# JCZ404/Semi-DETR

Hardware: AMD Instinct MI355X
Metric: images/sec/node DINO-R50 SSOD step (hot path: MSDA fwd/bwd + Hungarian + EMA/pseudo-label) (higher is better)
Workload: dtype f32

## Files before the change

include/semidetr_hip.h:

```cpp
#ifndef SEMIDETR_HIP_H
#define SEMIDETR_HIP_H

#include <stddef.h>
#include <stdint.h>

#ifdef __cplusplus
extern "C" {
#endif

#define SEMIDETR_OK 0
#define SEMIDETR_E_BADARG (-1)
#define SEMIDETR_E_TOOLARGE (-2)
#define SEMIDETR_E_NODEVICE (-3)

#define SEMIDETR_ABI_VERSION 7

int semidetr_abi_version(void);
const char *semidetr_last_error(void);

#define SEMIDETR_MSDA_QUERIES_ARE_PIXELS 1
#define SEMIDETR_MSDA_POLICY_SLOT(s) (((s) & 0xff) << 8)
#define SEMIDETR_MSDA_FIXED_FORWARD 2
#define SEMIDETR_MSDA_GATHER_WINDOW (1 << 16)
#define SEMIDETR_MSDA_GATHER_PATCH (1 << 17)
int semidetr_msda_forward_f32(void *stream, const float *value, const int64_t *spatial_shapes,
                              const int64_t *level_start, const float *sampling_loc,
                              const float *attn_weight, int batch, int spatial_size, int num_heads,
                              int channels, int num_levels, int num_query, int num_point, int flags, float *out);
int semidetr_msda_forward_f64(void *stream, const double *value, const int64_t *spatial_shapes,
                              const int64_t *level_start, const double *sampling_loc,
                              const double *attn_weight, int batch, int spatial_size, int num_heads,
                              int channels, int num_levels, int num_query, int num_point, double *out);
int semidetr_msda_backward_f32(void *stream, const float *grad_out, const float *value,
                               const int64_t *spatial_shapes, const int64_t *level_start,
                               const float *sampling_loc, const float *attn_weight, int batch,
                               int spatial_size, int num_heads, int channels, int num_levels,
                               int num_query, int num_point, int flags, float *grad_value,
                               float *grad_sampling_loc, float *grad_attn_weight);
int semidetr_msda_backward_f64(void *stream, const double *grad_out, const double *value,
                               const int64_t *spatial_shapes, const int64_t *level_start,
                               const double *sampling_loc, const double *attn_weight, int batch,
                               int spatial_size, int num_heads, int channels, int num_levels,
                               int num_query, int num_point, double *grad_value,
                               double *grad_sampling_loc, double *grad_attn_weight);

int semidetr_msda_fused_forward_f32(void *stream, const float *value, const int64_t *spatial_shapes,
                                    const int64_t *level_start, const float *reference_points, int ref_dim,
                                    const float *sampling_offsets, const float *attn_logits,
                                    const unsigned char *padding_mask, const int *mask_extents, int batch,
                                    int spatial_size, int num_heads, int channels, int num_levels,
                                    int num_query, int num_point, int flags, float *out);
int semidetr_msda_fused_backward_f32(void *stream, const float *grad_out, const float *value,
                                     const int64_t *spatial_shapes, const int64_t *level_start,
                                     const float *reference_points, int ref_dim,
                                     const float *sampling_offsets, const float *attn_logits,
                                     const unsigned char *padding_mask, const int *mask_extents, int batch,
                                     int spatial_size, int num_heads, int channels, int num_levels,
                                     int num_query, int num_point, int flags, float *grad_value,
                                     float *grad_sampling_offsets, float *grad_attn_logits);
int semidetr_msda_forward_f32_v2(void *stream, const float *value, const int64_t *spatial_shapes,
                                 const int64_t *level_start, const float *sampling_loc,
                                 const float *attn_weight, int batch, int spatial_size, int num_heads,
                                 int channels, int num_levels, int num_query, int num_point, int flags, float *out,
                                 const int64_t *host_spatial_shapes);
int semidetr_msda_backward_f32_v2(void *stream, const float *grad_out, const float *value,
                                  const int64_t *spatial_shapes, const int64_t *level_start,
                                  const float *sampling_loc, const float *attn_weight, int batch,
                                  int spatial_size, int num_heads, int channels, int num_levels,
                                  int num_query, int num_point, int flags, float *grad_value,
                                  float *grad_sampling_loc, float *grad_attn_weight, const int64_t *host_spatial_shapes);
int semidetr_msda_fused_forward_f32_v2(void *stream, const float *value, const int64_t *spatial_shapes,
                                       const int64_t *level_start, const float *reference_points, int ref_dim,
                                       const float *sampling_offsets, const float *attn_logits,
                                       const unsigned char *padding_mask, const int *mask_extents, int batch,
                                       int spatial_size, int num_heads, int channels, int num_levels,
                                       int num_query, int num_point, int flags, float *out,
                                       const int64_t *host_spatial_shapes);
int semidetr_msda_fused_backward_f32_v2(void *stream, const float *grad_out, const float *value,
                                        const int64_t *spatial_shapes, const int64_t *level_start,
                                        const float *reference_points, int ref_dim,
                                        const float *sampling_offsets, const float *attn_logits,
                                        const unsigned char *padding_mask, const int *mask_extents, int batch,
                                        int spatial_size, int num_heads, int channels, int num_levels,
                                        int num_query, int num_point, int flags, float *grad_value,
                                        float *grad_sampling_offsets, float *grad_attn_logits,
                                        const int64_t *host_spatial_shapes);
int semidetr_msda_mask_extents(void *stream, const unsigned char *padding_mask, const int64_t *spatial_shapes,
                               const int64_t *level_start, int batch, int spatial_size, int num_levels, int *extents);

int semidetr_msda_set_forward_policy(int policy);
int semidetr_msda_forward_policy_state(int *policy, int *mode, float *far_fraction, unsigned *updates);
int semidetr_msda_forward_policy_state_slot(int slot, int *policy, int *mode, float *far_fraction, unsigned *updates);
int semidetr_msda_gather_choice(int slot);

#define SEMIDETR_MSDA_GRID_FORWARD 0
#define SEMIDETR_MSDA_GRID_GATHER 1
#define SEMIDETR_MSDA_GRID_SCATTER 2
int semidetr_msda_set_region_grid(int kernel, int nry, int nrx);
int semidetr_msda_region_grid_query(int kernel, const int64_t *host_spatial_shapes, int num_levels, int batch, int num_heads,
                                    int num_cus, int *grid6);

const char *semidetr_msda_last_kernels(void);

#define SEMIDETR_H16_FP16 0
#define SEMIDETR_H16_BF16 1
int semidetr_msda_forward_h16(void *stream, int dtype, const void *value, const int64_t *spatial_shapes,
                              const int64_t *level_start, const float *sampling_loc, const float *attn_weight,
                              int batch, int spatial_size, int num_heads, int channels, int num_levels, int num_query,
                              int num_point, void *out);
size_t semidetr_msda_backward_h16_workspace_bytes(int batch, int spatial_size, int num_heads, int channels);
int semidetr_msda_backward_h16(void *stream, int dtype, const void *grad_out, const void *value,
                               const int64_t *spatial_shapes, const int64_t *level_start, const float *sampling_loc,
                               const float *attn_weight, int batch, int spatial_size, int num_heads, int channels,
                               int num_levels, int num_query, int num_point, void *workspace, void *grad_value,
                               float *grad_sampling_loc, float *grad_attn_weight);
int semidetr_msda_fused_forward_h16(void *stream, int dtype, const void *value, const int64_t *spatial_shapes,
                                    const int64_t *level_start, const float *reference_points, int ref_dim,
                                    const void *sampling_offsets, const void *attn_logits, int prologue_type,
                                    const unsigned char *padding_mask, int batch, int spatial_size, int num_heads,
                                    int channels, int num_levels, int num_query, int num_point, void *out);
int semidetr_msda_fused_backward_h16(void *stream, int dtype, const void *grad_out, const void *value,
                                     const int64_t *spatial_shapes, const int64_t *level_start,
                                     const float *reference_points, int ref_dim, const void *sampling_offsets,
                                     const void *attn_logits, int prologue_type, const unsigned char *padding_mask,
                                     int batch, int spatial_size, int num_heads, int channels, int num_levels,
                                     int num_query, int num_point, void *workspace, void *grad_value,
                                     void *grad_sampling_offsets, void *grad_attn_logits);
const char *semidetr_msda_h16_last_kernels(void);

typedef struct semidetr_cost_params {
    float cls_weight;
    float alpha;
    float gamma;
    float eps;
    float reg_weight;
    int   reg_xywh;
    float iou_weight;
    int   iou_giou;
    int   pred_xyxy;
} semidetr_cost_params;

int semidetr_match_cost_f32(void *stream, const float *bbox_pred, const float *cls_pred,
                            const float *gt_bboxes, const int64_t *gt_labels,
                            const int32_t *gt_offsets, const float *img_wh, int num_problems,
                            int num_query, int num_classes, int total_gt,
                            const semidetr_cost_params *params , float *cost);

int64_t semidetr_lsap_workspace_bytes(int num_problems, int num_query, int max_gt);
int semidetr_lsap_solve(void *stream, const float *cost, const int32_t *gt_offsets,
                        const int64_t *gt_labels, int num_problems, int num_query, int total_gt,
                        int max_gt, int64_t *match_row, int64_t *match_col,
                        int64_t *assigned_gt_inds, int64_t *assigned_labels, int32_t *status,
                        void *workspace);

int semidetr_build_targets(void *stream, const int64_t *assigned_gt_inds, const float *gt_bboxes,
                           const int64_t *gt_labels, const int32_t *gt_offsets, const float *img_wh,
                           int num_problems, int num_query, int64_t num_classes, int64_t *labels,
                           float *label_weights, float *bbox_targets, float *bbox_weights, int32_t *num_pos);

#define SEMIDETR_EMA_CHUNK 8192
int semidetr_ema_multi_f32(void *stream, float *const *teacher_ptrs, const float *const *student_ptrs,
                           const int64_t *numels, const int32_t *block_starts, int num_tensors,
                           int total_blocks, double momentum);
int semidetr_ema_flat_f32(void *stream, float *teacher, const float *student, int64_t numel,
                          double momentum);

int semidetr_pseudo_label_filter_f32(void *stream, const float *proposals, const int64_t *labels,
                                     const int32_t *prop_offsets, const int32_t *prop_counts,
                                     int num_images, float *out_boxes,
                                     int64_t *out_labels, float *out_scores, int32_t *out_keep_idx,
                                     int32_t *out_count, float *out_thr);

size_t semidetr_nms_workspace_bytes(int batch, int num_query, int num_classes);
int semidetr_pseudo_nms_f32(void *stream, const float *cls_logits, const float *bbox_pred, const float *img_hw,
                            int batch, int num_query, int num_classes, float score_thr, float iou_thr,
                            int max_per_img, void *workspace, size_t workspace_bytes, float *out_dets,
                            int64_t *out_labels, int32_t *out_count);

int semidetr_transform_bboxes_f32(void *stream, const float *boxes, int box_stride, const int32_t *box_offsets,
                                  const int32_t *box_counts, int num_images, int max_boxes_per_image,
                                  const float *matrices, const float *out_hw, float *out_boxes);

int semidetr_o2m_assign_f32(void *stream, const float *bbox_pred, const float *cls_prob, const float *gt_bboxes,
                            const int64_t *gt_labels, const int32_t *gt_offsets, const float *img_wh,
                            int num_problems, int num_query, int num_classes, int total_gt,
                            int max_gt_per_problem, int candidate_topk, int dynamic_k, float alpha, float beta,
                            int64_t *gt_inds, int64_t *labels, float *max_overlaps, float *assign_metrics,
                            int64_t *labels_full, float *bbox_targets, float *norm_metrics);

size_t semidetr_tal_loss_workspace_bytes(void);
int semidetr_tal_loss_f32(void *stream, const float *logits, const int64_t *labels, const float *metrics,
                          int64_t num_rows, int num_classes, float gamma, int input_is_prob, void *workspace,
                          float *loss_sum, float *grad_logits);

#define SEMIDETR_GMM_COVARIANCE_DIAG 1
int semidetr_gmm_match_costs_f32(void *stream, const float *cost, const int32_t *gt_offsets, const int32_t *pair_offsets,
                                 const int64_t *rows, const int64_t *cols, int num_images, int num_query, int num_pairs,
                                 int capacity, float *out_seg, int32_t *out_count);
int semidetr_gmm_fit_f64(void *stream, const float *values, int64_t value_stride, const int32_t *counts,
                         int64_t count_stride, int num_segments, int capacity, int covariance_type, double reg_covar,
                         double tol, int max_iter, float *out_thr, int32_t *out_labels, double *out_scores,
                         int32_t *out_info);
int semidetr_gmm_double_filter_f32(void *stream, const float *seg_costs, const int32_t *pair_offsets, const int64_t *cols,
                                   const float *thr, const float *gt_bboxes, const int64_t *gt_labels,
                                   const float *gt_scores, const float *det_bboxes, const int64_t *det_labels,
                                   const float *det_scores, const int32_t *gt_offsets, int num_images, int max_gt,
                                   float base_thr, int slot, float *out_base_boxes, int64_t *out_base_labels,
                                   float *out_base_scores, float *out_gmm_boxes, int64_t *out_gmm_labels,
                                   float *out_gmm_scores, float *out_det_boxes, int64_t *out_det_labels,
                                   float *out_det_scores, int32_t *out_counts);

#define SEMIDETR_SET_LOSS_MATCHED 0
#define SEMIDETR_SET_LOSS_DN 1
#define SEMIDETR_SET_LOSS_WARMUP 2
#define SEMIDETR_SET_LOSS_MAX_SEGMENTS 3
#define SEMIDETR_SET_LOSS_MAX_LAYERS 64
#define SEMIDETR_SET_LOSS_NUM_STATS 10
#define SEMIDETR_SET_LOSS_NUM_TERMS 5
typedef struct semidetr_set_loss_segment {
    int kind, num_layers, num_images, num_query, num_classes;
    const float *logits;
    int64_t logit_stride[3];
    const float *boxes;
    int64_t box_stride[3];
    const int64_t *labels;
    const float *label_weights, *bbox_targets, *bbox_weights, *metrics;
    const int32_t *gt_offsets;
    const float *gt_boxes;
    const int64_t *gt_labels;
    int single_pad, dn_groups;
    const float *img_wh;
    float alpha, gamma, cls_weight, l1_weight, iou_weight, iou_eps, bg_cls_weight;
    int sync_cls;
    float *grad_logits, *grad_boxes;
} semidetr_set_loss_segment;
int64_t semidetr_set_loss_workspace_bytes(const semidetr_set_loss_segment *segs, int num_segments);
int semidetr_set_loss_forward_f32(void *stream, const semidetr_set_loss_segment *segs, int num_segments, void *workspace,
                                  int64_t workspace_bytes, double *stats, float *norms, float *losses, float *scales);
int semidetr_set_loss_finalize_f32(void *stream, const semidetr_set_loss_segment *segs, int num_segments,
                                   const double *stats, const float *norms_local, const float *norms_reduced,
                                   float *losses, float *scales);
int semidetr_set_loss_backward_f32(void *stream, const semidetr_set_loss_segment *segs, int num_segments,
                                   const float *scales, const float *grad_out);

#define SEMIDETR_DN_MAX_IMAGES 64
#define SEMIDETR_DN_NOISE_COLS 10
typedef struct semidetr_dn_layout {
    int num_images, single_pad, groups;
    int32_t offsets[SEMIDETR_DN_MAX_IMAGES + 1];
} semidetr_dn_layout;
typedef struct semidetr_dn_build {
    semidetr_dn_layout dn, cons;
    int32_t src_counts[SEMIDETR_DN_MAX_IMAGES];
    const int64_t *labels[SEMIDETR_DN_MAX_IMAGES];
    const float *boxes[SEMIDETR_DN_MAX_IMAGES];
    int box_stride, num_known;
    const float *label_weight;
    int num_embeddings, hidden_dim, num_classes, num_queries;
    const float *noise, *image_noise;
    float label_noise_threshold, box_noise_scale;
    float *query_label, *query_bbox;
    int64_t *known_bid, *map_known_indice, *noised_labels, *pad_mask;
    const float *cons_rows;
    float *cons_label;
    unsigned char *attn_mask;
} semidetr_dn_build;
typedef struct semidetr_dn_consistency {
    semidetr_dn_layout cons;
    int32_t src_counts[SEMIDETR_DN_MAX_IMAGES];
    const float *pseudo_boxes[SEMIDETR_DN_MAX_IMAGES];
    const float *det_boxes[SEMIDETR_DN_MAX_IMAGES];
    int pseudo_stride, det_stride, num_known;
    float tgt_wh[SEMIDETR_DN_MAX_IMAGES][2], src_wh[SEMIDETR_DN_MAX_IMAGES][2];
    float *query_bbox, *known_bid;
    int64_t *map_known_indice;
    float *loss_weights, *rois;
    float loss_weight;
} semidetr_dn_consistency;
int semidetr_dn_build_f32(void *stream, const semidetr_dn_build *params );
int semidetr_dn_consistency_f32(void *stream, const semidetr_dn_consistency *params );
int semidetr_dn_label_backward_f32(void *stream, const float *grad_query_label, const int64_t *known_bid,
                                   const int64_t *map_known_indice, const int64_t *noised_labels, int num_known,
                                   int num_images, int pad_size, int hidden_dim, int num_embeddings, float *grad_weight);
int semidetr_dn_gather_rows_f32(void *stream, const semidetr_dn_layout *layout , const float *grad_label,
                                int hidden_dim, float *grad_rows);

#define SEMIDETR_QSEL_MAX_LEVELS 8
#define SEMIDETR_QSEL_MAX_K 4096
int semidetr_qsel_proposals_f32(void *stream, const float *memory, const unsigned char *padding_mask,
                                const int64_t *spatial_shapes_host, const int64_t *spatial_shapes_dev, int num_levels, int N,
                                int S, int D, float *output_memory, float *output_proposals, unsigned char *valid);
int semidetr_qsel_proposals_backward_f32(void *stream, const float *grad_output_memory, const unsigned char *valid, int N, int S,
                                         int D, float *grad_memory);
size_t semidetr_qsel_topk_workspace_bytes(int N, int S);
int semidetr_qsel_topk_f32(void *stream, const float *logits, int N, int S, int C, int k, void *workspace,
                           size_t workspace_bytes, int64_t *indices, int32_t *inverse);
int semidetr_qsel_gather_f32(void *stream, const int64_t *indices, const float *coord, const float *proposals,
                             const float *memory, int N, int S, int k, int D, float *refpoint, float *init_box, float *tgt,
                             float *ref_enc);
int semidetr_qsel_gather_backward_f32(void *stream, const int32_t *inverse, const float *grad_refpoint, const float *grad_tgt,
                                      const float *grad_ref_enc, const float *ref_enc, int N, int S, int k, int D,
                                      float *grad_coord, float *grad_memory);

#define SEMIDETR_DET_MAX_K 2048
size_t semidetr_det_workspace_bytes(int batch, int num_query, int num_classes, int k);
int semidetr_det_decode_f32(void *stream, const float *cls_logits, const float *bbox_pred, const float *img_hw,
                            const float *scale_factor , int batch, int num_query,
                            int num_classes, int k, void *workspace, size_t workspace_bytes, float *out_dets ,
                            int64_t *out_labels , float *out_dets_by_class ,
                            int32_t *out_class_offsets );

#define SEMIDETR_CONSIS_MAX_LAYERS 16
typedef struct semidetr_consis_layer {
    const float *v1, *v2;
    int64_t v1_stride[2], v2_stride[2];
    float *grad_v1;
} semidetr_consis_layer;
typedef struct semidetr_consis_loss {
    int num_layers, batch, num_query, dim, pad_size, num_known;
    int bid_is_int64;
    float scale, eps;
    const void *known_bid;
    const int64_t *map_known_indice;
    const float *loss_weights;
    semidetr_consis_layer layer[SEMIDETR_CONSIS_MAX_LAYERS];
} semidetr_consis_loss;
size_t semidetr_consis_loss_workspace_bytes(int num_layers, int num_known, int batch, int pad_size);
int semidetr_consis_loss_forward_f32(void *stream, const semidetr_consis_loss *params , void *workspace,
                                     size_t workspace_bytes, float *losses);
int semidetr_consis_loss_backward_f32(void *stream, const semidetr_consis_loss *params , const void *workspace,
                                      size_t workspace_bytes, const float *grad_losses);

typedef struct semidetr_self_attn {
    int batch, heads, head_dim, len_q, len_k;
    float scale;
    const float *q, *k, *v;
    int64_t q_stride[2], k_stride[2], v_stride[2];
    const uint8_t *mask;
    float *out, *lse;
    const float *grad_out;
    float *grad_q, *grad_k, *grad_v;
    int64_t gq_stride[2], gk_stride[2], gv_stride[2];
} semidetr_self_attn;
size_t semidetr_self_attn_workspace_bytes(int batch, int heads, int len_q, int len_k);
int semidetr_self_attn_forward_f32(void *stream, const semidetr_self_attn *params , void *workspace,
                                   size_t workspace_bytes);
int semidetr_self_attn_backward_f32(void *stream, const semidetr_self_attn *params , void *workspace,
                                    size_t workspace_bytes);

typedef struct semidetr_self_attn_h16 {
    int batch, heads, head_dim, len_q, len_k;
    float scale;
    int type;
    const void *q, *k, *v;
    int64_t q_stride[2], k_stride[2], v_stride[2];
    const uint8_t *mask;
    void *out;
    float *lse;
    const void *grad_out;
    void *grad_q, *grad_k, *grad_v;
    int64_t gq_stride[2], gk_stride[2], gv_stride[2];
} semidetr_self_attn_h16;
int semidetr_self_attn_forward_h16(void *stream, const semidetr_self_attn_h16 *params , void *workspace,
                                   size_t workspace_bytes);
int semidetr_self_attn_backward_h16(void *stream, const semidetr_self_attn_h16 *params , void *workspace,
                                    size_t workspace_bytes);

typedef struct semidetr_add_norm {
    int rows0, rows1, dim;
    float eps;
    const float *x, *residual, *pos;
    const float *gy, *gq;
    int64_t x_stride[2], residual_stride[2], pos_stride[2], gy_stride[2], gq_stride[2];
    const float *weight, *bias;
    float *y, *q;
    float *mean, *rstd;
    float *grad_x, *grad_weight, *grad_bias;
} semidetr_add_norm;
size_t semidetr_add_norm_workspace_bytes(int64_t rows);
int semidetr_add_norm_forward_f32(void *stream, const semidetr_add_norm *params , void *workspace,
                                  size_t workspace_bytes);
int semidetr_add_norm_backward_f32(void *stream, const semidetr_add_norm *params , void *workspace,
                                   size_t workspace_bytes);

#define SEMIDETR_ROW_F32 0
#define SEMIDETR_ROW_FP16 1
#define SEMIDETR_ROW_BF16 2
typedef struct semidetr_add_norm_mixed {
    int rows0, rows1, dim;
    float eps;
    const void *x, *residual, *pos;
    const void *gy, *gq;
    int64_t x_stride[2], residual_stride[2], pos_stride[2], gy_stride[2], gq_stride[2];
    const float *weight, *bias;
    void *y, *q;
    float *mean, *rstd;
    void *grad_x, *grad_residual, *grad_pos;
    float *grad_weight, *grad_bias;
    int x_type, residual_type, pos_type, gy_type, gq_type;
    int y_type, q_type, grad_x_type, grad_residual_type, grad_pos_type;
} semidetr_add_norm_mixed;
int semidetr_add_norm_forward_mixed(void *stream, const semidetr_add_norm_mixed *params , void *workspace,
                                    size_t workspace_bytes);
int semidetr_add_norm_backward_mixed(void *stream, const semidetr_add_norm_mixed *params , void *workspace,
                                     size_t workspace_bytes);

#define SEMIDETR_GN_MAX_LEVELS 8
typedef struct semidetr_gn_tokens {
    int batch, levels, channels, groups;
    float eps;
    int64_t hw[SEMIDETR_GN_MAX_LEVELS], start[SEMIDETR_GN_MAX_LEVELS];
    int64_t tokens_per_image;
    const void *x[SEMIDETR_GN_MAX_LEVELS];
    int64_t x_batch_stride[SEMIDETR_GN_MAX_LEVELS];
    const float *weight[SEMIDETR_GN_MAX_LEVELS], *bias[SEMIDETR_GN_MAX_LEVELS];
    void *grad_x[SEMIDETR_GN_MAX_LEVELS];
    float *grad_weight[SEMIDETR_GN_MAX_LEVELS], *grad_bias[SEMIDETR_GN_MAX_LEVELS];
    void *tokens, *q;
    const void *pos, *gy, *gq;
    int64_t pos_stride[2], gy_stride[2], gq_stride[2];
    float *mean, *rstd;
    int x_type, out_type, pos_type;
} semidetr_gn_tokens;
size_t semidetr_gn_tokens_workspace_bytes(const semidetr_gn_tokens *params , int for_backward);
int semidetr_gn_tokens_forward(void *stream, const semidetr_gn_tokens *params , void *workspace,
                               size_t workspace_bytes);
int semidetr_gn_tokens_backward(void *stream, const semidetr_gn_tokens *params , void *workspace,
                                size_t workspace_bytes);

#define SEMIDETR_REF_MAX_SEGMENTS 8
#define SEMIDETR_REF_MAX_LEVELS 8
#define SEMIDETR_REF_NONE 0
#define SEMIDETR_REF_SIGMOID 1
#define SEMIDETR_REF_REFINE 2
typedef struct semidetr_ref_segment {
    int rows0, rows1;
    const void *delta, *ref;
    int64_t delta_stride[2], ref_stride[2];
    void *new_ref;
    int64_t new_ref_stride[2];
    const void *g_new;
    int64_t g_new_stride[2];
    void *g_delta, *g_ref;
} semidetr_ref_segment;
typedef struct semidetr_ref_points {
    int width, mode, num_segments, levels;
    float eps;
    int delta_type, ref_type, out_type;
    const float *valid_ratios;
    const float *dim_t;
    float *ref_input;
    float *embed;
    const float *g_ref_input, *g_embed;
    semidetr_ref_segment segment[SEMIDETR_REF_MAX_SEGMENTS];
} semidetr_ref_points;
int semidetr_ref_points_forward(void *stream, const semidetr_ref_points *params );
int semidetr_ref_points_backward(void *stream, const semidetr_ref_points *params );

#ifdef __cplusplus
}
#endif
#endif
```

semi-detr_amd/_lib.py:

```python
import contextlib
import ctypes
import os

import torch

_HERE = os.path.dirname(os.path.abspath(__file__))
EXPERIMENTS = os.environ.get("SEMIDETR_EXPERIMENTS", "0") not in ("", "0")
LIB_PATH = os.path.join(_HERE, "csrc", "libsemidetr_hip_exp.so" if EXPERIMENTS else "libsemidetr_hip.so")

c_void_p, c_int, c_int64, c_double = ctypes.c_void_p, ctypes.c_int, ctypes.c_int64, ctypes.c_double
c_float, c_size_t, POINTER = ctypes.c_float, ctypes.c_size_t, ctypes.POINTER

CONSTANTS = {
    "SEMIDETR_ABI_VERSION": 7,
    "SEMIDETR_EMA_CHUNK": 8192,
    "SEMIDETR_GMM_COVARIANCE_DIAG": 1,
    "SEMIDETR_SET_LOSS_MATCHED": 0, "SEMIDETR_SET_LOSS_DN": 1, "SEMIDETR_SET_LOSS_WARMUP": 2,
    "SEMIDETR_SET_LOSS_MAX_LAYERS": 64, "SEMIDETR_SET_LOSS_NUM_STATS": 10, "SEMIDETR_SET_LOSS_NUM_TERMS": 5,
    "SEMIDETR_DN_MAX_IMAGES": 64, "SEMIDETR_DN_NOISE_COLS": 10,
    "SEMIDETR_QSEL_MAX_LEVELS": 8, "SEMIDETR_QSEL_MAX_K": 4096,
    "SEMIDETR_DET_MAX_K": 2048,
    "SEMIDETR_CONSIS_MAX_LAYERS": 16,
}
ROW_TYPES = {"SEMIDETR_ROW_F32": 0, "SEMIDETR_ROW_FP16": 1, "SEMIDETR_ROW_BF16": 2}
_DN_IMAGES, _CONSIS_LAYERS = CONSTANTS["SEMIDETR_DN_MAX_IMAGES"], CONSTANTS["SEMIDETR_CONSIS_MAX_LAYERS"]
_STRIDE2 = c_int64 * 2


def _f(ctype, names):
    return [(n, ctype) for n in names.split()]


class CostParams(ctypes.Structure):
    _fields_ = (_f(c_float, "cls_weight alpha gamma eps reg_weight") + _f(c_int, "reg_xywh") + _f(c_float, "iou_weight")
                + _f(c_int, "iou_giou pred_xyxy"))


class SetLossSegment(ctypes.Structure):
    _fields_ = (_f(c_int, "kind num_layers num_images num_query num_classes")
                + _f(c_void_p, "logits") + _f(c_int64 * 3, "logit_stride") + _f(c_void_p, "boxes") + _f(c_int64 * 3, "box_stride")
                + _f(c_void_p, "labels label_weights bbox_targets bbox_weights metrics gt_offsets gt_boxes gt_labels")
                + _f(c_int, "single_pad dn_groups") + _f(c_void_p, "img_wh")
                + _f(c_float, "alpha gamma cls_weight l1_weight iou_weight iou_eps bg_cls_weight") + _f(c_int, "sync_cls")
                + _f(c_void_p, "grad_logits grad_boxes"))


class DnLayout(ctypes.Structure):
    _fields_ = _f(c_int, "num_images single_pad groups") + _f(ctypes.c_int32 * (_DN_IMAGES + 1), "offsets")


class DnBuild(ctypes.Structure):
    _fields_ = (_f(DnLayout, "dn cons") + _f(ctypes.c_int32 * _DN_IMAGES, "src_counts") + _f(c_void_p * _DN_IMAGES, "labels boxes")
                + _f(c_int, "box_stride num_known") + _f(c_void_p, "label_weight")
                + _f(c_int, "num_embeddings hidden_dim num_classes num_queries") + _f(c_void_p, "noise image_noise")
                + _f(c_float, "label_noise_threshold box_noise_scale")
                + _f(c_void_p, "query_label query_bbox known_bid map_known_indice noised_labels pad_mask cons_rows cons_label "
                               "attn_mask"))


class DnConsistency(ctypes.Structure):
    _fields_ = (_f(DnLayout, "cons") + _f(ctypes.c_int32 * _DN_IMAGES, "src_counts")
                + _f(c_void_p * _DN_IMAGES, "pseudo_boxes det_boxes") + _f(c_int, "pseudo_stride det_stride num_known")
                + _f(c_float * 2 * _DN_IMAGES, "tgt_wh src_wh")
                + _f(c_void_p, "query_bbox known_bid map_known_indice loss_weights rois") + _f(c_float, "loss_weight"))


class ConsisLayer(ctypes.Structure):
    _fields_ = _f(c_void_p, "v1 v2") + _f(_STRIDE2, "v1_stride v2_stride") + _f(c_void_p, "grad_v1")


class ConsisLoss(ctypes.Structure):
    _fields_ = (_f(c_int, "num_layers batch num_query dim pad_size num_known bid_is_int64") + _f(c_float, "scale eps")
                + _f(c_void_p, "known_bid map_known_indice loss_weights") + _f(ConsisLayer * _CONSIS_LAYERS, "layer"))


class SelfAttn(ctypes.Structure):
    _fields_ = (_f(c_int, "batch heads head_dim len_q len_k") + _f(c_float, "scale") + _f(c_void_p, "q k v")
                + _f(_STRIDE2, "q_stride k_stride v_stride") + _f(c_void_p, "mask out lse grad_out grad_q grad_k grad_v")
                + _f(_STRIDE2, "gq_stride gk_stride gv_stride"))


class SelfAttnH16(ctypes.Structure):
    _fields_ = (_f(c_int, "batch heads head_dim len_q len_k") + _f(c_float, "scale") + _f(c_int, "type") + _f(c_void_p, "q k v")
                + _f(_STRIDE2, "q_stride k_stride v_stride") + _f(c_void_p, "mask out lse grad_out grad_q grad_k grad_v")
                + _f(_STRIDE2, "gq_stride gk_stride gv_stride"))


class AddNorm(ctypes.Structure):
    _fields_ = (_f(c_int, "rows0 rows1 dim") + _f(c_float, "eps") + _f(c_void_p, "x residual pos gy gq")
                + _f(_STRIDE2, "x_stride residual_stride pos_stride gy_stride gq_stride")
                + _f(c_void_p, "weight bias y q mean rstd grad_x grad_weight grad_bias"))


class AddNormMixed(ctypes.Structure):
    _fields_ = (_f(c_int, "rows0 rows1 dim") + _f(c_float, "eps") + _f(c_void_p, "x residual pos gy gq")
                + _f(_STRIDE2, "x_stride residual_stride pos_stride gy_stride gq_stride")
                + _f(c_void_p, "weight bias y q mean rstd grad_x grad_residual grad_pos grad_weight grad_bias")
                + _f(c_int, "x_type residual_type pos_type gy_type gq_type y_type q_type grad_x_type grad_residual_type "
                            "grad_pos_type"))


GN_MAX_LEVELS = 8
_GN_I64, _GN_PTR = c_int64 * GN_MAX_LEVELS, c_void_p * GN_MAX_LEVELS


class GnTokens(ctypes.Structure):
    _fields_ = (_f(c_int, "batch levels channels groups") + _f(c_float, "eps") + _f(_GN_I64, "hw start")
                + _f(c_int64, "tokens_per_image") + _f(_GN_PTR, "x") + _f(_GN_I64, "x_batch_stride")
                + _f(_GN_PTR, "weight bias grad_x grad_weight grad_bias") + _f(c_void_p, "tokens q pos gy gq")
                + _f(_STRIDE2, "pos_stride gy_stride gq_stride") + _f(c_void_p, "mean rstd") + _f(c_int, "x_type out_type pos_type"))


REF_MAX_SEGMENTS, REF_MAX_LEVELS = 8, 8
REF_MODES = {"SEMIDETR_REF_NONE": 0, "SEMIDETR_REF_SIGMOID": 1, "SEMIDETR_REF_REFINE": 2}


class RefSegment(ctypes.Structure):
    _fields_ = (_f(c_int, "rows0 rows1") + _f(c_void_p, "delta ref") + _f(_STRIDE2, "delta_stride ref_stride")
                + _f(c_void_p, "new_ref") + _f(_STRIDE2, "new_ref_stride") + _f(c_void_p, "g_new") + _f(_STRIDE2, "g_new_stride")
                + _f(c_void_p, "g_delta g_ref"))


class RefPoints(ctypes.Structure):
    _fields_ = (_f(c_int, "width mode num_segments levels") + _f(c_float, "eps") + _f(c_int, "delta_type ref_type out_type")
                + _f(c_void_p, "valid_ratios dim_t ref_input embed g_ref_input g_embed")
                + _f(RefSegment * REF_MAX_SEGMENTS, "segment"))


STRUCTS = {"semidetr_cost_params": CostParams, "semidetr_set_loss_segment": SetLossSegment, "semidetr_dn_layout": DnLayout,
           "semidetr_dn_build": DnBuild, "semidetr_dn_consistency": DnConsistency, "semidetr_consis_layer": ConsisLayer,
           "semidetr_consis_loss": ConsisLoss, "semidetr_self_attn": SelfAttn, "semidetr_self_attn_h16": SelfAttnH16,
           "semidetr_add_norm": AddNorm,
           "semidetr_add_norm_mixed": AddNormMixed, "semidetr_gn_tokens": GnTokens,
           "semidetr_ref_segment": RefSegment, "semidetr_ref_points": RefPoints}
_SEGS, _WORK = POINTER(SetLossSegment), [c_void_p, c_size_t]

_MSDA_FWD = [c_void_p] * 6 + [c_int] * 7 + [c_void_p]
_MSDA_BWD = [c_void_p] * 7 + [c_int] * 7 + [c_void_p] * 3
_MSDA_FWD_F32 = [c_void_p] * 6 + [c_int] * 8 + [c_void_p]
_MSDA_BWD_F32 = [c_void_p] * 7 + [c_int] * 8 + [c_void_p] * 3

SIGNATURES = {
    "semidetr_abi_version": (c_int, []),
    "semidetr_last_error": (ctypes.c_char_p, []),
    "semidetr_msda_forward_f32": (c_int, _MSDA_FWD_F32),
    "semidetr_msda_forward_f64": (c_int, _MSDA_FWD),
    "semidetr_msda_backward_f32": (c_int, _MSDA_BWD_F32),
    "semidetr_msda_backward_f64": (c_int, _MSDA_BWD),
    "semidetr_msda_fused_forward_f32": (c_int, [c_void_p] * 5 + [c_int] + [c_void_p] * 4 + [c_int] * 8 + [c_void_p]),
    "semidetr_msda_fused_backward_f32": (c_int, [c_void_p] * 6 + [c_int] + [c_void_p] * 4 + [c_int] * 8 + [c_void_p] * 3),
    "semidetr_msda_forward_f32_v2": (c_int, _MSDA_FWD_F32 + [c_void_p]),
    "semidetr_msda_backward_f32_v2": (c_int, _MSDA_BWD_F32 + [c_void_p]),
    "semidetr_msda_fused_forward_f32_v2": (c_int, [c_void_p] * 5 + [c_int] + [c_void_p] * 4 + [c_int] * 8 + [c_void_p] * 2),
    "semidetr_msda_fused_backward_f32_v2": (c_int, [c_void_p] * 6 + [c_int] + [c_void_p] * 4 + [c_int] * 8 + [c_void_p] * 4),
    "semidetr_msda_mask_extents": (c_int, [c_void_p] * 4 + [c_int] * 3 + [c_void_p]),
    "semidetr_msda_last_kernels": (ctypes.c_char_p, []),
    "semidetr_msda_forward_h16": (c_int, [c_void_p, c_int] + [c_void_p] * 5 + [c_int] * 7 + [c_void_p]),
    "semidetr_msda_backward_h16_workspace_bytes": (c_size_t, [c_int] * 4),
    "semidetr_msda_backward_h16": (c_int, [c_void_p, c_int] + [c_void_p] * 6 + [c_int] * 7 + [c_void_p] * 4),
    "semidetr_msda_fused_forward_h16": (c_int, [c_void_p, c_int] + [c_void_p] * 4 + [c_int] + [c_void_p] * 2 + [c_int, c_void_p] +
                                        [c_int] * 7 + [c_void_p]),
    "semidetr_msda_fused_backward_h16": (c_int, [c_void_p, c_int] + [c_void_p] * 5 + [c_int] + [c_void_p] * 2 + [c_int, c_void_p] +
                                         [c_int] * 7 + [c_void_p] * 4),
    "semidetr_msda_h16_last_kernels": (ctypes.c_char_p, []),
    "semidetr_msda_set_forward_policy": (c_int, [c_int]),
    "semidetr_msda_forward_policy_state": (c_int, [c_void_p] * 4),
    "semidetr_msda_forward_policy_state_slot": (c_int, [c_int] + [c_void_p] * 4),
    "semidetr_msda_gather_choice": (c_int, [c_int]),
    "semidetr_msda_set_region_grid": (c_int, [c_int] * 3),
    "semidetr_msda_region_grid_query": (c_int, [c_int, c_void_p] + [c_int] * 4 + [c_void_p]),
    "semidetr_match_cost_f32": (c_int, [c_void_p] * 7 + [c_int] * 4 + [POINTER(CostParams), c_void_p]),
    "semidetr_lsap_workspace_bytes": (c_int64, [c_int, c_int, c_int]),
    "semidetr_lsap_solve": (c_int, [c_void_p] * 4 + [c_int] * 4 + [c_void_p] * 6),
    "semidetr_build_targets": (c_int, [c_void_p] * 6 + [c_int, c_int, c_int64] + [c_void_p] * 5),
    "semidetr_ema_multi_f32": (c_int, [c_void_p] * 5 + [c_int, c_int, c_double]),
    "semidetr_ema_flat_f32": (c_int, [c_void_p, c_void_p, c_void_p, c_int64, c_double]),
    "semidetr_pseudo_label_filter_f32": (c_int, [c_void_p] * 5 + [c_int] + [c_void_p] * 6),
    "semidetr_nms_workspace_bytes": (c_size_t, [c_int, c_int, c_int]),
    "semidetr_pseudo_nms_f32": (c_int, [c_void_p] * 4 + [c_int] * 3 + [c_float, c_float, c_int, c_void_p,
                                                                       c_size_t] + [c_void_p] * 3),
    "semidetr_o2m_assign_f32": (c_int, [c_void_p] * 7 + [c_int] * 7 + [c_float, c_float] + [c_void_p] * 7),
    "semidetr_tal_loss_workspace_bytes": (c_size_t, []),
    "semidetr_tal_loss_f32": (c_int, [c_void_p] * 4 + [c_int64, c_int, c_float, c_int] + [c_void_p] * 3),
    "semidetr_transform_bboxes_f32": (c_int, [c_void_p, c_void_p, c_int, c_void_p, c_void_p, c_int, c_int] + [c_void_p] * 3),
    "semidetr_gmm_match_costs_f32": (c_int, [c_void_p] * 6 + [c_int] * 4 + [c_void_p] * 2),
    "semidetr_gmm_fit_f64": (c_int, [c_void_p, c_void_p, c_int64, c_void_p, c_int64] + [c_int] * 3 + [c_double, c_double, c_int]
                             + [c_void_p] * 4),
    "semidetr_gmm_double_filter_f32": (c_int, [c_void_p] * 12 + [c_int, c_int, c_float, c_int] + [c_void_p] * 10),
    "semidetr_set_loss_workspace_bytes": (c_int64, [_SEGS, c_int]),
    "semidetr_set_loss_forward_f32": (c_int, [c_void_p, _SEGS, c_int, c_void_p, c_int64] + [c_void_p] * 4),
    "semidetr_set_loss_finalize_f32": (c_int, [c_void_p, _SEGS, c_int] + [c_void_p] * 5),
    "semidetr_set_loss_backward_f32": (c_int, [c_void_p, _SEGS, c_int, c_void_p, c_void_p]),
    "semidetr_dn_build_f32": (c_int, [c_void_p, POINTER(DnBuild)]),
    "semidetr_dn_consistency_f32": (c_int, [c_void_p, POINTER(DnConsistency)]),
    "semidetr_dn_label_backward_f32": (c_int, [c_void_p] * 5 + [c_int] * 5 + [c_void_p]),
    "semidetr_dn_gather_rows_f32": (c_int, [c_void_p, POINTER(DnLayout), c_void_p, c_int, c_void_p]),
    "semidetr_qsel_proposals_f32": (c_int, [c_void_p] * 5 + [c_int] * 4 + [c_void_p] * 3),
    "semidetr_qsel_proposals_backward_f32": (c_int, [c_void_p] * 3 + [c_int] * 3 + [c_void_p]),
    "semidetr_qsel_topk_workspace_bytes": (c_size_t, [c_int, c_int]),
    "semidetr_qsel_topk_f32": (c_int, [c_void_p, c_void_p] + [c_int] * 4 + [c_void_p, c_size_t, c_void_p, c_void_p]),
    "semidetr_qsel_gather_f32": (c_int, [c_void_p] * 5 + [c_int] * 4 + [c_void_p] * 4),
    "semidetr_qsel_gather_backward_f32": (c_int, [c_void_p] * 6 + [c_int] * 4 + [c_void_p] * 2),
    "semidetr_det_workspace_bytes": (c_size_t, [c_int] * 4),
    "semidetr_det_decode_f32": (c_int, [c_void_p] * 5 + [c_int] * 4 + [c_void_p, c_size_t] + [c_void_p] * 4),
    "semidetr_consis_loss_workspace_bytes": (c_size_t, [c_int] * 4),
    "semidetr_consis_loss_forward_f32": (c_int, [c_void_p, POINTER(ConsisLoss)] + _WORK + [c_void_p]),
    "semidetr_consis_loss_backward_f32": (c_int, [c_void_p, POINTER(ConsisLoss)] + _WORK + [c_void_p]),
    "semidetr_self_attn_workspace_bytes": (c_size_t, [c_int] * 4),
    "semidetr_self_attn_forward_f32": (c_int, [c_void_p, POINTER(SelfAttn)] + _WORK),
    "semidetr_self_attn_backward_f32": (c_int, [c_void_p, POINTER(SelfAttn)] + _WORK),
    "semidetr_self_attn_forward_h16": (c_int, [c_void_p, POINTER(SelfAttnH16)] + _WORK),
    "semidetr_self_attn_backward_h16": (c_int, [c_void_p, POINTER(SelfAttnH16)] + _WORK),
    "semidetr_add_norm_workspace_bytes": (c_size_t, [c_int64]),
    "semidetr_add_norm_forward_f32": (c_int, [c_void_p, POINTER(AddNorm)] + _WORK),
    "semidetr_add_norm_backward_f32": (c_int, [c_void_p, POINTER(AddNorm)] + _WORK),
    "semidetr_add_norm_forward_mixed": (c_int, [c_void_p, POINTER(AddNormMixed)] + _WORK),
    "semidetr_add_norm_backward_mixed": (c_int, [c_void_p, POINTER(AddNormMixed)] + _WORK),
    "semidetr_gn_tokens_workspace_bytes": (c_size_t, [POINTER(GnTokens), c_int]),
    "semidetr_gn_tokens_forward": (c_int, [c_void_p, POINTER(GnTokens)] + _WORK),
    "semidetr_gn_tokens_backward": (c_int, [c_void_p, POINTER(GnTokens)] + _WORK),
    "semidetr_ref_points_forward": (c_int, [c_void_p, POINTER(RefPoints)]),
    "semidetr_ref_points_backward": (c_int, [c_void_p, POINTER(RefPoints)]),
}

EXPERIMENT_SIGNATURES = {
    "semidetr_msda_set_variant": (None, [c_int, c_int]),
    "semidetr_debug_counters": (c_int, [c_void_p, c_int]),
    "semidetr_stream_copy_f32": (c_int, [c_void_p, c_void_p, c_void_p, c_int64, c_int]),
}

_lib = None


class NativeLibraryError(RuntimeError):
    pass


def lib():
    global _lib
    if _lib is None:
        if not os.path.exists(LIB_PATH):
            raise NativeLibraryError(
                f"{LIB_PATH} not found: build it with `python -c 'import __graft_entry__ as g; g.build()'` "
                "or `make -C semi-detr_amd/csrc` (hipcc --offload-arch=gfx950). There is no CPU fallback.")
        handle = ctypes.CDLL(LIB_PATH)
        table = dict(SIGNATURES, **EXPERIMENT_SIGNATURES) if EXPERIMENTS else SIGNATURES
        for name, (res, args) in table.items():
            fn = getattr(handle, name)
            fn.restype, fn.argtypes = res, args
        _lib = handle
    return _lib


def check(rc, what):
    if rc != 0:
        msg = lib().semidetr_last_error().decode(errors="replace")
        raise RuntimeError(f"{what} failed (code {rc}): {msg}")


def current_stream_ptr():
    return c_void_p(torch.cuda.current_stream().cuda_stream)


_NO_GUARD = contextlib.nullcontext()
_Tensor = torch.Tensor
_functions = {}


def device_guard(dev):
    if dev.index is None or dev.index == torch.cuda.current_device():
        return _NO_GUARD
    return torch.cuda.device(dev)


def ptr_args(args):
    return [c_void_p(a.data_ptr()) if isinstance(a, _Tensor) else a for a in args]


def _function(name):
    hit = _functions.get(name)
    if hit is not None and hit[0] is _lib:
        return hit[1]
    if name not in SIGNATURES and not (EXPERIMENTS and name in EXPERIMENT_SIGNATURES):
        raise AttributeError(f"{name} is not a function of the C ABI (_lib.SIGNATURES)")
    fn = getattr(lib(), name)
    _functions[name] = (_lib, fn)
    return fn


def calls(dev, *launches):
    fns = [_function(launch[0]) for launch in launches]
    with device_guard(dev):
        stream = c_void_p(torch.cuda.current_stream(dev).cuda_stream)
        for fn, launch in zip(fns, launches):
            rc = fn(stream, *ptr_args(launch[1:]))
            if rc:
                check(rc, launch[0])


def call(name, dev, *args):
    calls(dev, (name,) + args)


def small_to_device(values, dtype, dev):
    host = torch.tensor(values, dtype=dtype)
    if dev.type == "cuda":
        return host.pin_memory().to(dev, non_blocking=True)
    return host.to(dev)


def offsets(counts, dev):
    offs = [0]
    for c in counts:
        offs.append(offs[-1] + int(c))
    return offs, small_to_device(offs, torch.int32, dev)


def rows_f32(t):
    t = t.detach()
    if t.dtype != torch.float32:
        t = t.float()
    if t.stride(2) != 1 or t.data_ptr() % 16 or t.stride(0) % 4 or t.stride(1) % 4:
        t = t.contiguous()
    return t


def row_type(dtype):
    code = _ROW_TYPE_OF.get(dtype)
    if code is None:
        raise TypeError(f"rows of {dtype} are not built (float32, float16, bfloat16)")
    return code


_ROW_TYPE_OF = {torch.float32: ROW_TYPES["SEMIDETR_ROW_F32"], torch.float16: ROW_TYPES["SEMIDETR_ROW_FP16"],
                torch.bfloat16: ROW_TYPES["SEMIDETR_ROW_BF16"]}


def rows_native(t):
    t = t.detach()
    row_type(t.dtype)
    if t.stride(2) != 1 or t.data_ptr() % (16 if t.dtype == torch.float32 else 8) or t.stride(0) % 4 or t.stride(1) % 4:
        t = t.contiguous()
    return t


def set_rows(block, name, t, stride=None):
    if t is None:
        return
    setattr(block, name, t.data_ptr())
    st, strides = getattr(block, stride or name + "_stride"), t.stride()
    st[0], st[1] = strides[0], strides[1]


def cast(t, dtype):
    return t if t is None or t.dtype == dtype else t.to(dtype)


FORWARD_POLICIES = {"adaptive": 0, "patch": 1, "window": 2}


def set_forward_policy(policy):
    check(lib().semidetr_msda_set_forward_policy(FORWARD_POLICIES.get(policy, policy)), "semidetr_msda_set_forward_policy")


def forward_policy_state(slot=0):
    pol, mode, upd, frac = c_int(), c_int(), ctypes.c_uint(), c_float()
    check(lib().semidetr_msda_forward_policy_state_slot(int(slot), ctypes.byref(pol), ctypes.byref(mode), ctypes.byref(frac),
                                                        ctypes.byref(upd)), "semidetr_msda_forward_policy_state_slot")
    return {"policy": pol.value, "mode": mode.value, "far_fraction": frac.value, "updates": upd.value}


REGION_GRID_KERNELS = {"forward": 0, "gather": 1, "scatter": 2}


def set_region_grid(kernel, nry=0, nrx=0):
    check(lib().semidetr_msda_set_region_grid(REGION_GRID_KERNELS.get(kernel, kernel), int(nry), int(nrx)),
          "semidetr_msda_set_region_grid")


def region_grid(kernel, spatial_shapes, batch, num_heads, num_cus):
    flat = None if spatial_shapes is None else [int(v) for hw in spatial_shapes for v in hw]
    table = None if flat is None else (c_int64 * len(flat))(*flat)
    levels = 1 if flat is None else len(flat) // 2
    out = (c_int * 6)()
    check(lib().semidetr_msda_region_grid_query(REGION_GRID_KERNELS.get(kernel, kernel), table, levels, int(batch), int(num_heads),
                                                int(num_cus), out), "semidetr_msda_region_grid_query")
    return dict(zip(("nry", "nrx", "regions", "workgroups", "tail_split", "max_queries"), out))


def set_variant(fwd, bwd):
    if EXPERIMENTS:
        lib().semidetr_msda_set_variant(int(fwd), int(bwd))
    elif (fwd, bwd) != (0, 0):
        raise NativeLibraryError("kernel variants exist only in the experiments build: set SEMIDETR_EXPERIMENTS=1 "
                                 "(libsemidetr_hip_exp.so) before importing semi_detr_amd")
```

semi-detr_amd/csrc/lsap.hip:

```cpp
#include <hip/hip_runtime.h>

#include "common.h"

#pragma clang fp contract(off)

namespace {

constexpr double kInf = __builtin_huge_val();

struct Best {
    double low;
    int first;
    int last_un;
};

__device__ __forceinline__ Best combine(const Best &a, const Best &b)
{
    if (b.low < a.low) return b;
    if (a.low < b.low) return a;
    Best r = a;
    r.first = min(a.first, b.first);
    r.last_un = max(a.last_un, b.last_un);
    return r;
}

template <int CTRL>
__device__ __forceinline__ Best dpp_best(const Best &x)
{
    const unsigned long long lb = __builtin_bit_cast(unsigned long long, x.low);
    const int lo = __builtin_amdgcn_update_dpp(0, (int)(unsigned)lb, CTRL, 0xF, 0xF, true);
    const int hi = __builtin_amdgcn_update_dpp(0, (int)(unsigned)(lb >> 32), CTRL, 0xF, 0xF, true);
    Best o;
    o.low = __builtin_bit_cast(double, ((unsigned long long)(unsigned)hi << 32) | (unsigned)lo);
    o.first = __builtin_amdgcn_update_dpp(0, x.first, CTRL, 0xF, 0xF, true);
    o.last_un = __builtin_amdgcn_update_dpp(0, x.last_un, CTRL, 0xF, 0xF, true);
    return o;
}

__device__ __forceinline__ Best lane_best(const Best &x, int l)
{
    const unsigned long long lb = __builtin_bit_cast(unsigned long long, x.low);
    const unsigned lo = (unsigned)__builtin_amdgcn_readlane((int)(unsigned)lb, l);
    const unsigned hi = (unsigned)__builtin_amdgcn_readlane((int)(unsigned)(lb >> 32), l);
    Best o;
    o.low = __builtin_bit_cast(double, ((unsigned long long)hi << 32) | lo);
    o.first = __builtin_amdgcn_readlane(x.first, l);
    o.last_un = __builtin_amdgcn_readlane(x.last_un, l);
    return o;
}

__device__ __forceinline__ Best wave_best(Best x)
{
    x = combine(x, dpp_best<0xB1>(x));
    x = combine(x, dpp_best<0x4E>(x));
    x = combine(x, dpp_best<0x141>(x));
    x = combine(x, dpp_best<0x140>(x));
    const Best a = combine(lane_best(x, 0), lane_best(x, 16)), c = combine(lane_best(x, 32), lane_best(x, 48));
    return combine(a, c);
}

__device__ __forceinline__ int wave_sum_i(int v)
{
#pragma unroll
    for (int s = 32; s > 0; s >>= 1) v += __shfl_xor(v, s, 64);
    return v;
}

__host__ __device__ inline size_t align16(size_t x) { return (x + 15) & ~(size_t)15; }
__host__ __device__ inline size_t lsap_bytes(int ncmax, int nrmax)
{
    return align16((size_t)ncmax * 8) * 2 + align16((size_t)nrmax * 8) + align16((size_t)ncmax * 4) * 3 +
           align16((size_t)nrmax * 4) + align16((size_t)(nrmax + 1) * 4);
}

template <bool USE_LDS, bool COST_LDS = false>
__global__ __launch_bounds__(64) void lsap_kernel(
    const float *__restrict__ cost, const int32_t *__restrict__ gt_offsets,
    const int64_t *__restrict__ gt_labels, int Q, int ncmax, int nrmax, int64_t *__restrict__ match_row,
    int64_t *__restrict__ match_col, int64_t *__restrict__ gt_inds, int64_t *__restrict__ labels,
    int32_t *__restrict__ status, char *__restrict__ ws, size_t ws_stride)
{
    extern __shared__ double smem_d[];
    const int b = blockIdx.x, lane = threadIdx.x;
    const int g0 = gt_offsets[b], G = gt_offsets[b + 1] - g0;

    for (int q = lane; q < Q; q += 64) {
        if (gt_inds) gt_inds[(int64_t)b * Q + q] = 0;
        if (labels) labels[(int64_t)b * Q + q] = -1;
    }
    if (lane == 0) status[b] = 0;
    if (G <= 0 || Q <= 0) return;

    int po = 0;
    for (int bb = lane; bb < b; bb += 64) po += min(Q, gt_offsets[bb + 1] - gt_offsets[bb]);
    po = wave_sum_i(po);

    const bool tr = G < Q;
    const int nr = tr ? G : Q, nc = tr ? Q : G;
    const float *cb = cost + (int64_t)Q * g0;
    const int64_t si = tr ? Q : 1, sj = tr ? 1 : Q;

    char *base = USE_LDS ? reinterpret_cast<char *>(smem_d) : ws + (size_t)b * ws_stride;
    double *v = reinterpret_cast<double *>(base);       base += align16((size_t)ncmax * 8);
    double *spc = reinterpret_cast<double *>(base);     base += align16((size_t)ncmax * 8);
    double *u = reinterpret_cast<double *>(base);       base += align16((size_t)nrmax * 8);
    int *path = reinterpret_cast<int *>(base);          base += align16((size_t)ncmax * 4);
    int *row4col = reinterpret_cast<int *>(base);       base += align16((size_t)ncmax * 4);
    int *remaining = reinterpret_cast<int *>(base);     base += align16((size_t)ncmax * 4);
    int *col4row = reinterpret_cast<int *>(base);       base += align16((size_t)nrmax * 4);
    int *scanned = reinterpret_cast<int *>(base);       base += align16((size_t)(nrmax + 1) * 4);
    float *cl = reinterpret_cast<float *>(base);

    int bad = 0;
    {
        const int64_t total = (int64_t)nr * nc;
        auto check = [&](float c) { if (c != c || c == -__builtin_huge_valf()) bad = 1; };
        int64_t k = 0;
        if ((reinterpret_cast<uintptr_t>(cb) & 15) == 0) {
            const float4 *cb4 = reinterpret_cast<const float4 *>(cb);
            float4 *cl4 = reinterpret_cast<float4 *>(cl);
            const int64_t n4 = total / 4;
            for (int64_t k4 = lane; k4 < n4; k4 += 64 * 8) {
                float4 c[8];
#pragma unroll
                for (int t = 0; t < 8; ++t) c[t] = k4 + 64 * t < n4 ? cb4[k4 + 64 * t] : make_float4(0.f, 0.f, 0.f, 0.f);
#pragma unroll
                for (int t = 0; t < 8; ++t) {
                    check(c[t].x); check(c[t].y); check(c[t].z); check(c[t].w);
                    if (COST_LDS && k4 + 64 * t < n4) cl4[k4 + 64 * t] = c[t];
                }
            }
            k = n4 * 4;
        }
        for (k += lane; k < total; k += 64) {
            const float c = cb[k];
            check(c);
            if (COST_LDS) cl[k] = c;
        }
    }
    if (__any(bad)) {
        if (lane == 0) status[b] = 2;
        return;
    }

    for (int j = lane; j < nc; j += 64) { v[j] = 0.0; path[j] = -1; row4col[j] = -1; }
    for (int i = lane; i < nr; i += 64) { u[i] = 0.0; col4row[i] = -1; }
    __syncthreads();

    for (int cur = 0; cur < nr; ++cur) {
        for (int j = lane; j < nc; j += 64) { spc[j] = kInf; remaining[j] = nc - j - 1; }
        __syncthreads();
        int num_rem = nc, ns = 0, sink = -1, i = cur;
        double min_val = 0.0;
        while (sink == -1) {
            const double ui = u[i];
            const float *crow = (COST_LDS ? cl : cb) + (int64_t)i * si;
            Best best = {kInf, 0x7fffffff, -1};
            constexpr int kScan = 16;
            for (int it0 = lane; it0 < num_rem; it0 += 64 * kScan) {
                int jj[kScan];
                double cc[kScan], vv[kScan], ss[kScan];
                int rr[kScan];
#pragma unroll
                for (int t = 0; t < kScan; ++t) jj[t] = it0 + 64 * t < num_rem ? remaining[it0 + 64 * t] : -1;
#pragma unroll
                for (int t = 0; t < kScan; ++t) {
                    const int j = jj[t] < 0 ? 0 : jj[t];
                    cc[t] = (double)crow[(int64_t)j * sj];
                    vv[t] = v[j];
                    ss[t] = spc[j];
                    rr[t] = row4col[j];
                }
#pragma unroll
                for (int t = 0; t < kScan; ++t) {
                    if (jj[t] < 0) break;
                    const int it = it0 + 64 * t, j = jj[t];
                    const double r = min_val + cc[t] - ui - vv[t];
                    double s = ss[t];
                    if (r < s) { path[j] = i; spc[j] = r; s = r; }
                    const bool un = rr[t] == -1;
                    if (s < best.low) { best.low = s; best.first = it; best.last_un = un ? it : -1; }
                    else if (s == best.low && un) best.last_un = it;
                }
            }
            best = wave_best(best);
            min_val = best.low;
            if (min_val == kInf) {
                if (lane == 0) status[b] = 1;
                return;
            }
            const int idx = best.last_un >= 0 ? best.last_un : best.first;
            const int j = remaining[idx];
            const int r4c = row4col[j];
            __syncthreads();
            if (lane == 0) { scanned[ns] = j; remaining[idx] = remaining[num_rem - 1]; }
            ++ns; --num_rem;
            if (r4c == -1) sink = j; else i = r4c;
            __syncthreads();
        }
        if (lane == 0) u[cur] += min_val;
        for (int t = lane; t < ns; t += 64) {
            const int j = scanned[t];
            const double d = min_val - spc[j];
            if (j != sink) u[row4col[j]] += d;
            v[j] -= d;
        }
        __syncthreads();
        if (lane == 0) {
            int j = sink;
            for (;;) {
                const int ii = path[j];
                row4col[j] = ii;
                const int t = col4row[ii];
                col4row[ii] = j;
                j = t;
                if (ii == cur) break;
            }
        }
        __syncthreads();
    }

    for (int i = lane; i < nr; i += 64) {
        const int c = col4row[i];
        int q, g, rank;
        if (tr) {
            q = c; g = i; rank = 0;
            for (int k = 0; k < nr; ++k) rank += col4row[k] < c;
        } else {
            q = i; g = c; rank = i;
        }
        if (match_row) match_row[po + rank] = q;
        if (match_col) match_col[po + rank] = g;
        if (gt_inds) gt_inds[(int64_t)b * Q + q] = g + 1;
        if (labels) labels[(int64_t)b * Q + q] = gt_labels[g0 + g];
    }
}

constexpr size_t kLdsLimit = 64 * 1024;
constexpr size_t kLdsBig = 150 * 1024;

#pragma clang fp contract(off)
__global__ __launch_bounds__(256) void build_targets_kernel(
    const int64_t *__restrict__ gt_inds, const float *__restrict__ gt_bboxes, const int64_t *__restrict__ gt_labels,
    const int32_t *__restrict__ gt_offsets, const float *__restrict__ img_wh, int Q, int64_t num_classes,
    int64_t *__restrict__ labels, float *__restrict__ label_weights, float *__restrict__ bbox_targets,
    float *__restrict__ bbox_weights, int32_t *__restrict__ num_pos)
{
    const int b = blockIdx.y, q = blockIdx.x * 256 + threadIdx.x;
    bool pos = false;
    if (q < Q) {
        const int64_t o = (int64_t)b * Q + q;
        const int64_t gi = gt_inds[o];
        pos = gi > 0;
        float4 t = make_float4(0.f, 0.f, 0.f, 0.f);
        int64_t lab = num_classes;
        if (pos) {
            const int64_t g = gt_offsets[b] + gi - 1;
            const float4 bx = *reinterpret_cast<const float4 *>(gt_bboxes + g * 4);
            const float w = img_wh[2 * b], h = img_wh[2 * b + 1];
            const float x1 = bx.x / w, y1 = bx.y / h, x2 = bx.z / w, y2 = bx.w / h;
            t = make_float4((x1 + x2) / 2, (y1 + y2) / 2, x2 - x1, y2 - y1);
            lab = gt_labels[g];
        }
        labels[o] = lab;
        label_weights[o] = 1.f;
        *reinterpret_cast<float4 *>(bbox_targets + o * 4) = t;
        const float wgt = pos ? 1.f : 0.f;
        *reinterpret_cast<float4 *>(bbox_weights + o * 4) = make_float4(wgt, wgt, wgt, wgt);
    }
    const int n = __popcll(__ballot(pos));
    if ((threadIdx.x & 63) == 0 && n) atomicAdd(&num_pos[b], n);
}

}

extern "C" int64_t semidetr_lsap_workspace_bytes(int num_problems, int num_query, int max_gt)
{
    if (num_problems <= 0 || num_query <= 0 || max_gt <= 0) return 0;
    const int ncmax = num_query > max_gt ? num_query : max_gt;
    const int nrmax = num_query < max_gt ? num_query : max_gt;
    const size_t per = lsap_bytes(ncmax, nrmax);
    return per <= kLdsLimit ? 0 : (int64_t)(per * (size_t)num_problems);
}

extern "C" int semidetr_lsap_solve(void *stream, const float *cost, const int32_t *gt_offsets,
                                   const int64_t *gt_labels, int num_problems, int num_query, int total_gt,
                                   int max_gt, int64_t *match_row, int64_t *match_col,
                                   int64_t *assigned_gt_inds, int64_t *assigned_labels, int32_t *status,
                                   void *workspace)
{
    SEMIDETR_REQUIRE(num_problems >= 0 && num_query >= 0 && total_gt >= 0 && max_gt >= 0 && max_gt <= total_gt,
                     SEMIDETR_E_BADARG, "lsap: bad sizes (B=%d Q=%d sumG=%d maxG=%d)", num_problems, num_query,
                     total_gt, max_gt);
    if (num_problems == 0) return SEMIDETR_OK;
    SEMIDETR_REQUIRE(gt_offsets && status, SEMIDETR_E_BADARG, "lsap: null gt_offsets/status");
    SEMIDETR_REQUIRE(total_gt == 0 || num_query == 0 || cost, SEMIDETR_E_BADARG, "lsap: null cost");
    SEMIDETR_REQUIRE(!assigned_labels || total_gt == 0 || gt_labels, SEMIDETR_E_BADARG, "lsap: null gt_labels");
    const int ncmax = num_query > max_gt ? num_query : max_gt;
    const int nrmax = num_query < max_gt ? num_query : max_gt;
    const size_t per = lsap_bytes(ncmax > 0 ? ncmax : 1, nrmax > 0 ? nrmax : 1);
    hipStream_t st = semidetr::as_stream(stream);
    const size_t cost_bytes = (size_t)max_gt * (size_t)num_query * sizeof(float);
    if (per <= kLdsLimit && per + cost_bytes <= kLdsBig) {
        if (int rc = semidetr::allow_big_lds(&lsap_kernel<true, true>, kLdsBig, "lsap")) return rc;
        hipLaunchKernelGGL((lsap_kernel<true, true>), dim3(num_problems), dim3(64), per + cost_bytes, st, cost, gt_offsets,
                           gt_labels, num_query, ncmax, nrmax, match_row, match_col, assigned_gt_inds,
                           assigned_labels, status, (char *)nullptr, (size_t)0);
    } else if (per <= kLdsLimit) {
        hipLaunchKernelGGL(lsap_kernel<true>, dim3(num_problems), dim3(64), per, st, cost, gt_offsets,
                           gt_labels, num_query, ncmax, nrmax, match_row, match_col, assigned_gt_inds,
                           assigned_labels, status, (char *)nullptr, (size_t)0);
    } else {
        SEMIDETR_REQUIRE(workspace, SEMIDETR_E_BADARG, "lsap: workspace of %lld bytes required",
                         (long long)(per * (size_t)num_problems));
        hipLaunchKernelGGL(lsap_kernel<false>, dim3(num_problems), dim3(64), 0, st, cost, gt_offsets,
                           gt_labels, num_query, ncmax, nrmax, match_row, match_col, assigned_gt_inds,
                           assigned_labels, status, (char *)workspace, per);
    }
    return semidetr::launch_status("lsap_kernel");
}

extern "C" int semidetr_build_targets(void *stream, const int64_t *assigned_gt_inds, const float *gt_bboxes,
                                      const int64_t *gt_labels, const int32_t *gt_offsets, const float *img_wh,
                                      int num_problems, int num_query, int64_t num_classes, int64_t *labels,
                                      float *label_weights, float *bbox_targets, float *bbox_weights,
                                      int32_t *num_pos)
{
    SEMIDETR_REQUIRE(num_problems >= 0 && num_query >= 0, SEMIDETR_E_BADARG, "build_targets: negative sizes");
    if (num_problems == 0) return SEMIDETR_OK;
    SEMIDETR_REQUIRE(assigned_gt_inds && gt_offsets && img_wh && labels && label_weights && bbox_targets &&
                         bbox_weights && num_pos,
                     SEMIDETR_E_BADARG, "build_targets: null pointer argument");
    SEMIDETR_REQUIRE(num_problems <= 65535, SEMIDETR_E_TOOLARGE, "build_targets: more than 65535 problems");
    hipStream_t st = semidetr::as_stream(stream);
    hipError_t e = hipMemsetAsync(num_pos, 0, sizeof(int32_t) * (size_t)num_problems, st);
    if (e != hipSuccess) return semidetr::fail((int)e, "build_targets memset: %s", hipGetErrorString(e));
    if (num_query == 0) return SEMIDETR_OK;
    hipLaunchKernelGGL(build_targets_kernel, dim3((num_query + 255) / 256, num_problems), dim3(256), 0, st,
                       assigned_gt_inds, gt_bboxes, gt_labels, gt_offsets, img_wh, num_query, num_classes, labels,
                       label_weights, bbox_targets, bbox_weights, num_pos);
    return semidetr::launch_status("build_targets_kernel");
}
```

semi-detr_amd/csrc/match_cost.hip:

```cpp
#include <hip/hip_runtime.h>

#include "common.h"

#pragma clang fp contract(off)

namespace {

__device__ __forceinline__ float pow_gamma(float x, float gamma)
{
    return gamma == 2.0f ? x * x : powf(x, gamma);
}

__global__ __launch_bounds__(256) void match_cost_kernel(
    const float *__restrict__ bbox_pred, const float *__restrict__ cls_pred,
    const float *__restrict__ gt_bboxes, const int64_t *__restrict__ gt_labels,
    const int32_t *__restrict__ gt_offsets, const float *__restrict__ img_wh, int Q, int C,
    semidetr_cost_params prm, float *__restrict__ cost)
{
    const int b = blockIdx.y;
    const int g0 = gt_offsets[b], G = gt_offsets[b + 1] - g0;
    const int q = blockIdx.x * 256 + threadIdx.x;
    if (G <= 0 || q >= Q) return;
    const float img_w = img_wh[2 * b], img_h = img_wh[2 * b + 1];
    const float4 bp = *reinterpret_cast<const float4 *>(bbox_pred + ((int64_t)b * Q + q) * 4);
    float cx = bp.x, cy = bp.y, bw = bp.z, bh = bp.w;
    float nx0 = cx - 0.5f * bw, ny0 = cy - 0.5f * bh, nx1 = cx + 0.5f * bw, ny1 = cy + 0.5f * bh;
    if (prm.pred_xyxy) {
        nx0 = bp.x; ny0 = bp.y; nx1 = bp.z; ny1 = bp.w;
        cx = (nx0 + nx1) / 2; cy = (ny0 + ny1) / 2; bw = nx1 - nx0; bh = ny1 - ny0;
    }
    const float x0 = nx0 * img_w, y0 = ny0 * img_h, x1 = nx1 * img_w, y1 = ny1 * img_h;
    const float area1 = (x1 - x0) * (y1 - y0);
    const float *cls_row = cls_pred + ((int64_t)b * Q + q) * C;
    float *out = cost + (int64_t)Q * g0 + q;
    for (int j = 0; j < G; ++j) {
        const float4 gt = *reinterpret_cast<const float4 *>(gt_bboxes + (int64_t)(g0 + j) * 4);
        const int label = (int)gt_labels[g0 + j];
        const float x = (unsigned)label < (unsigned)C ? cls_row[label] : __builtin_nanf("");
        const float p = 1.0f / (1.0f + expf(-x));
        const float neg = -logf(1.0f - p + prm.eps) * (1.0f - prm.alpha) * pow_gamma(p, prm.gamma);
        const float pos = -logf(p + prm.eps) * prm.alpha * pow_gamma(1.0f - p, prm.gamma);
        const float c_cls = (pos - neg) * prm.cls_weight;
        const float n0 = gt.x / img_w, n1 = gt.y / img_h, n2 = gt.z / img_w, n3 = gt.w / img_h;
        float l1;
        if (prm.reg_xywh) {
            const float t0 = (n0 + n2) / 2, t1 = (n1 + n3) / 2, t2 = n2 - n0, t3 = n3 - n1;
            l1 = fabsf(cx - t0) + fabsf(cy - t1) + fabsf(bw - t2) + fabsf(bh - t3);
        } else {
            l1 = fabsf(nx0 - n0) + fabsf(ny0 - n1) + fabsf(nx1 - n2) + fabsf(ny1 - n3);
        }
        const float c_reg = l1 * prm.reg_weight;
        const float area2 = (gt.z - gt.x) * (gt.w - gt.y);
        const float ow = fmaxf(fminf(x1, gt.z) - fmaxf(x0, gt.x), 0.0f);
        const float oh = fmaxf(fminf(y1, gt.w) - fmaxf(y0, gt.y), 0.0f);
        const float overlap = ow * oh;
        const float uni = fmaxf(area1 + area2 - overlap, 1e-6f);
        float iou = overlap / uni;
        if (prm.iou_giou) {
            const float ew = fmaxf(fmaxf(x1, gt.z) - fminf(x0, gt.x), 0.0f);
            const float eh = fmaxf(fmaxf(y1, gt.w) - fminf(y0, gt.y), 0.0f);
            const float earea = fmaxf(ew * eh, 1e-6f);
            iou = iou - (earea - uni) / earea;
        }
        const float c_iou = -iou * prm.iou_weight;
        out[(int64_t)j * Q] = c_cls + c_reg + c_iou;
    }
}

}

extern "C" int semidetr_match_cost_f32(void *stream, const float *bbox_pred, const float *cls_pred,
                                       const float *gt_bboxes, const int64_t *gt_labels,
                                       const int32_t *gt_offsets, const float *img_wh, int num_problems,
                                       int num_query, int num_classes, int total_gt,
                                       const semidetr_cost_params *params, float *cost)
{
    SEMIDETR_REQUIRE(num_problems >= 0 && num_query >= 0 && num_classes > 0 && total_gt >= 0,
                     SEMIDETR_E_BADARG, "match_cost: bad sizes (B=%d Q=%d C=%d sumG=%d)", num_problems,
                     num_query, num_classes, total_gt);
    SEMIDETR_REQUIRE(params, SEMIDETR_E_BADARG, "match_cost: null params");
    if (num_problems == 0 || num_query == 0 || total_gt == 0) return SEMIDETR_OK;
    SEMIDETR_REQUIRE(bbox_pred && cls_pred && gt_bboxes && gt_labels && gt_offsets && img_wh && cost,
                     SEMIDETR_E_BADARG, "match_cost: null pointer argument");
    SEMIDETR_REQUIRE(num_problems <= 65535, SEMIDETR_E_TOOLARGE, "match_cost: more than 65535 problems");
    SEMIDETR_REQUIRE((int64_t)num_query * total_gt < INT32_MAX, SEMIDETR_E_TOOLARGE, "match_cost: matrix too large");
    SEMIDETR_REQUIRE((((uintptr_t)bbox_pred | (uintptr_t)gt_bboxes) & 15) == 0, SEMIDETR_E_BADARG,
                     "match_cost: bbox_pred / gt_bboxes must be 16-byte aligned");
    const dim3 grid((num_query + 255) / 256, num_problems);
    hipLaunchKernelGGL(match_cost_kernel, grid, dim3(256), 0, semidetr::as_stream(stream), bbox_pred,
                       cls_pred, gt_bboxes, gt_labels, gt_offsets, img_wh, num_query, num_classes, *params,
                       cost);
    return semidetr::launch_status("match_cost_kernel");
}
```

semi-detr_amd/csrc/nms.hip:

```cpp
#include <hip/hip_runtime.h>

#include "common.h"

#pragma clang fp contract(off)

#include "select.h"

namespace {

using semidetr::bitonic_desc;
using semidetr::kHistStride;
using semidetr::order_key;
using semidetr::sigmoidf_;

__device__ __forceinline__ float4 decode_box(const float *bp, float img_h, float img_w)
{
    const float cx = bp[0], cy = bp[1], w = bp[2], h = bp[3];
    const float x1 = (cx - 0.5f * w) * img_w, y1 = (cy - 0.5f * h) * img_h;
    const float x2 = (cx + 0.5f * w) * img_w, y2 = (cy + 0.5f * h) * img_h;
    return make_float4(fminf(fmaxf(x1, 0.f), img_w), fminf(fmaxf(y1, 0.f), img_h), fminf(fmaxf(x2, 0.f), img_w),
                       fminf(fmaxf(y2, 0.f), img_h));
}

__device__ __forceinline__ bool iou_gt(const float4 a, const float4 b, float thr)
{
    const float left = fmaxf(a.x, b.x), right = fminf(a.z, b.z);
    const float top = fmaxf(a.y, b.y), bottom = fminf(a.w, b.w);
    const float width = right - left, height = bottom - top;
    if (!(width > 0.f && height > 0.f)) return false;
    const float inter = width * height;
    const float sa = (a.z - a.x) * (a.w - a.y), sb = (b.z - b.x) * (b.w - b.y);
    return inter / (sa + sb - inter) > thr;
}

struct Workspace {
    float4 *boxes;
    float *maxc;
    int *count;
    unsigned long long *keys;
};

__host__ __device__ inline size_t align256(size_t v) { return (v + 255) & ~(size_t)255; }

inline size_t workspace_bytes(int B, int Q, int C)
{
    return align256(sizeof(float4) * (size_t)B * Q) + align256(sizeof(float) * (size_t)B) +
           align256(sizeof(int) * (size_t)B) + align256(sizeof(unsigned long long) * (size_t)B * Q * C);
}

inline Workspace carve(void *ws, int B, int Q, int C)
{
    char *p = static_cast<char *>(ws);
    Workspace w;
    w.boxes = reinterpret_cast<float4 *>(p); p += align256(sizeof(float4) * (size_t)B * Q);
    w.maxc = reinterpret_cast<float *>(p); p += align256(sizeof(float) * (size_t)B);
    w.count = reinterpret_cast<int *>(p); p += align256(sizeof(int) * (size_t)B);
    w.keys = reinterpret_cast<unsigned long long *>(p);
    (void)C;
    return w;
}

constexpr int kPrepQueries = 16;
__global__ __launch_bounds__(256) void nms_prepare_kernel(const float *__restrict__ logits,
                                                          const float *__restrict__ bbox_pred,
                                                          const float *__restrict__ img_hw, int Q, int C,
                                                          float score_thr, Workspace ws)
{
    __shared__ float red[4];
    const int b = blockIdx.y, lane = threadIdx.x & 63, wv = threadIdx.x >> 6;
    const float img_h = img_hw[2 * b], img_w = img_hw[2 * b + 1];
    float mx = 0.f;
    for (int r = wv; r < kPrepQueries; r += 4) {
        const int q = blockIdx.x * kPrepQueries + r;
        if (q >= Q) break;
        const float4 box = decode_box(bbox_pred + ((size_t)b * Q + q) * 4, img_h, img_w);
        const float *lr = logits + ((size_t)b * Q + q) * C;
        bool any = false;
        for (int c = lane; c < C; c += 64) any |= sigmoidf_(lr[c]) > score_thr;
        if (lane == 0) ws.boxes[(size_t)b * Q + q] = box;
        if (__ballot(any) != 0ull) mx = fmaxf(mx, fmaxf(fmaxf(box.x, box.y), fmaxf(box.z, box.w)));
    }
    if (lane == 0) red[wv] = mx;
    __syncthreads();
    if (threadIdx.x == 0) {
        mx = fmaxf(fmaxf(red[0], red[1]), fmaxf(red[2], red[3]));
        if (mx > 0.f) atomicMax(reinterpret_cast<int *>(ws.maxc) + b, __float_as_int(mx));
    }
}

template <int NP2, int NW>
__global__ __launch_bounds__(64 * NW) void nms_class_kernel(const float *__restrict__ logits, int Q, int C,
                                                            float score_thr, float iou_thr, Workspace ws)
{
    constexpr int NT = 64 * NW;
    __shared__ unsigned long long keys[NP2];
    __shared__ float4 ob[NP2];
    __shared__ float4 kb[NP2];
    __shared__ unsigned long long s_hit[NW], s_row[NW][64];
    __shared__ int s_base, s_n;
    const int c = blockIdx.x, b = blockIdx.y, tid = threadIdx.x, lane = tid & 63, wv = tid >> 6;
    const unsigned long long lt = (1ull << lane) - 1ull;
    if (tid == 0) s_n = 0;
    __syncthreads();
    for (int q0 = 0; q0 < Q; q0 += NT) {
        const int q = q0 + tid;
        unsigned long long key = 0;
        if (q < Q) {
            const float x = logits[((size_t)b * Q + q) * C + c];
            if (sigmoidf_(x) > score_thr)
                key = ((unsigned long long)order_key(x) << 32) | (unsigned)(0xFFFFFFFFu - (unsigned)q);
        }
        const unsigned long long mask = __ballot(key != 0);
        int base = 0;
        if (lane == 0 && mask) base = atomicAdd(&s_n, __popcll(mask));
        base = __shfl(base, 0, 64);
        if (key) keys[base + __popcll(mask & lt)] = key;
    }
    __syncthreads();
    const int n = s_n;
    int n2 = 64;
    while (n2 < n) n2 <<= 1;
    for (int i = n + tid; i < n2; i += NT) keys[i] = 0;
    bitonic_desc<NT>(keys, n2);
    if (n == 0) return;
    const float off = (float)c * (ws.maxc[b] + 1.0f);
    for (int i = tid; i < n; i += NT) {
        const int q = (int)(0xFFFFFFFFu - (unsigned)(keys[i] & 0xFFFFFFFFull));
        const float4 bx = ws.boxes[(size_t)b * Q + q];
        ob[i] = make_float4(bx.x + off, bx.y + off, bx.z + off, bx.w + off);
    }
    __syncthreads();
    int m = 0;
    for (int i0 = 0; i0 < n; i0 += 64) {
        const int j = i0 + lane;
        const bool valid = j < n;
        const float4 bj = ob[valid ? j : 0];
        bool hit = false;
        const int share = ((m + NW - 1) / NW + 7) & ~7;
        int k = wv * share;
        const int kend = min(m, k + share);
        for (; k + 8 <= kend; k += 8) {
            float4 kk[8];
#pragma unroll
            for (int u = 0; u < 8; ++u) kk[u] = kb[k + u];
#pragma unroll
            for (int u = 0; u < 8; ++u) hit |= iou_gt(kk[u], bj, iou_thr);
        }
        for (; k < kend; ++k) hit |= iou_gt(kb[k], bj, iou_thr);
        unsigned long long row = 0;
        const int cn = n - i0 < 64 ? n - i0 : 64;
        int i = wv * (64 / NW);
        const int iend = min(cn, i + 64 / NW);
        for (; i + 8 <= iend; i += 8) {
            float4 kk[8];
#pragma unroll
            for (int u = 0; u < 8; ++u) kk[u] = ob[i0 + i + u];
#pragma unroll
            for (int u = 0; u < 8; ++u)
                if (i + u < lane && iou_gt(kk[u], bj, iou_thr)) row |= 1ull << (i + u);
        }
        for (; i < iend; ++i)
            if (i < lane && iou_gt(ob[i0 + i], bj, iou_thr)) row |= 1ull << i;
        unsigned long long hits = __ballot(hit);
        if (NW > 1) {
            if (lane == 0) s_hit[wv] = hits;
            s_row[wv][lane] = row;
            __syncthreads();
            hits = 0;
            row = 0;
#pragma unroll
            for (int w = 0; w < NW; ++w) {
                hits |= s_hit[w];
                row |= s_row[w][lane];
            }
        }
        const bool alive = valid && !((hits >> lane) & 1ull);
        unsigned long long cand = __ballot(alive), kept = 0;
        const unsigned row_lo = (unsigned)row, row_hi = (unsigned)(row >> 32);
        while (cand) {
            const int ci = __ffsll((long long)cand) - 1;
            cand &= cand - 1;
            const unsigned long long ri = ((unsigned long long)(unsigned)__builtin_amdgcn_readlane((int)row_hi, ci) << 32) |
                                          (unsigned)__builtin_amdgcn_readlane((int)row_lo, ci);
            if ((ri & kept) == 0) kept |= 1ull << ci;
        }
        const bool keep = wv == 0 && ((kept >> lane) & 1ull);
        const int total = __popcll(kept);
        if (keep) kb[m + __popcll(kept & lt)] = bj;
        if (tid == 0) s_base = total ? atomicAdd(&ws.count[b], total) : 0;
        __syncthreads();
        if (keep) {
            const unsigned q = 0xFFFFFFFFu - (unsigned)(keys[j] & 0xFFFFFFFFull);
            const unsigned flat = q * (unsigned)C + (unsigned)c;
            ws.keys[(size_t)b * Q * C + s_base + __popcll(kept & lt)] =
                (keys[j] & 0xFFFFFFFF00000000ull) | (unsigned)(0xFFFFFFFFu - flat);
        }
        m += total;
        __syncthreads();
    }
}

constexpr int kTopThreads = 1024, kTopCap = 2048;
constexpr int kHistCopies = 64;

__global__ __launch_bounds__(kTopThreads) void nms_topk_kernel(const float *__restrict__ logits, int Q, int C,
                                                               int max_num, Workspace ws, float *__restrict__ dets,
                                                               int64_t *__restrict__ labels, int32_t *__restrict__ out_count)
{
    __shared__ unsigned long long sel[kTopCap];
    __shared__ int hist[kHistCopies * kHistStride];
    __shared__ int bins[256];
    __shared__ int s_digit, s_remaining, s_matching, s_fill;
    const int b = blockIdx.x, tid = threadIdx.x;
    const int K = ws.count[b];
    const unsigned long long *keys = ws.keys + (size_t)b * Q * C;
    const int nout = K < max_num ? K : max_num;
    for (int i = tid; i < kTopCap; i += kTopThreads) sel[i] = 0;
    if (tid == 0) { s_fill = 0; s_remaining = nout; s_matching = K; }
    __syncthreads();
    if (K <= kTopCap) {
        for (int i = tid; i < K; i += kTopThreads) sel[i] = keys[i];
    } else {
        unsigned long long prefix = 0, mask = 0;
        for (int pass = 7; pass >= 0; --pass) {
            semidetr::histogram_pass<kTopThreads, kHistCopies>(hist, keys, K, prefix, mask, pass);
            semidetr::pick_digit<kTopThreads, kHistCopies>(hist, bins, &s_digit, &s_remaining, &s_matching);
            prefix |= (unsigned long long)s_digit << (8 * pass);
            mask |= 0xFFull << (8 * pass);
            if ((nout - s_remaining) + s_matching <= kTopCap) break;
        }
        for (int i = tid; i < K; i += kTopThreads) {
            const unsigned long long k = keys[i];
            if ((k & mask) >= prefix) sel[atomicAdd(&s_fill, 1)] = k;
        }
    }
    bitonic_desc<kTopThreads>(sel, kTopCap);
    for (int r = tid; r < nout; r += kTopThreads) {
        const unsigned flat = 0xFFFFFFFFu - (unsigned)(sel[r] & 0xFFFFFFFFull);
        const int q = (int)(flat / (unsigned)C), c = (int)(flat % (unsigned)C);
        const float4 bx = ws.boxes[(size_t)b * Q + q];
        float *o = dets + ((size_t)b * max_num + r) * 5;
        o[0] = bx.x; o[1] = bx.y; o[2] = bx.z; o[3] = bx.w;
        o[4] = sigmoidf_(logits[((size_t)b * Q + q) * C + c]);
        labels[(size_t)b * max_num + r] = c;
    }
    if (tid == 0) out_count[b] = nout;
}

__global__ __launch_bounds__(256) void transform_bboxes_kernel(const float *__restrict__ boxes, int box_stride,
                                                               const int32_t *__restrict__ offs,
                                                               const int32_t *__restrict__ counts,
                                                               const float *__restrict__ mats,
                                                               const float *__restrict__ out_hw,
                                                               float *__restrict__ out)
{
    const int b = blockIdx.y;
    const int p0 = offs[b], K = counts ? counts[b] : offs[b + 1] - p0;
    const int i = blockIdx.x * 256 + threadIdx.x;
    if (i >= K) return;
    const float *M = mats + 9 * b;
    const float *bx = boxes + (size_t)(p0 + i) * box_stride;
    const float px[4] = {bx[0], bx[2], bx[2], bx[0]}, py[4] = {bx[1], bx[1], bx[3], bx[3]};
    float minx = __builtin_huge_valf(), miny = minx, maxx = -minx, maxy = -minx;
#pragma unroll
    for (int k = 0; k < 4; ++k) {
        const float x = M[0] * px[k] + M[1] * py[k] + M[2];
        const float y = M[3] * px[k] + M[4] * py[k] + M[5];
        const float z = M[6] * px[k] + M[7] * py[k] + M[8];
        const float u = x / z, v = y / z;
        minx = fminf(minx, u); maxx = fmaxf(maxx, u);
        miny = fminf(miny, v); maxy = fmaxf(maxy, v);
    }
    const float oh = out_hw[2 * b], ow = out_hw[2 * b + 1];
    float *o = out + (size_t)(p0 + i) * 4;
    o[0] = fminf(fmaxf(minx, 0.f), ow);
    o[1] = fminf(fmaxf(miny, 0.f), oh);
    o[2] = fminf(fmaxf(maxx, 0.f), ow);
    o[3] = fminf(fmaxf(maxy, 0.f), oh);
}

}

extern "C" size_t semidetr_nms_workspace_bytes(int batch, int num_query, int num_classes)
{
    if (batch <= 0 || num_query <= 0 || num_classes <= 0) return 0;
    return workspace_bytes(batch, num_query, num_classes);
}

extern "C" int semidetr_pseudo_nms_f32(void *stream, const float *cls_logits, const float *bbox_pred,
                                       const float *img_hw, int batch, int num_query, int num_classes,
                                       float score_thr, float iou_thr, int max_per_img, void *workspace,
                                       size_t workspace_bytes_, float *out_dets, int64_t *out_labels,
                                       int32_t *out_count)
{
    const int B = batch, Q = num_query, C = num_classes;
    SEMIDETR_REQUIRE(B >= 0 && Q >= 0 && C >= 0, SEMIDETR_E_BADARG, "pseudo_nms: negative size");
    if (B == 0) return SEMIDETR_OK;
    SEMIDETR_REQUIRE(out_count, SEMIDETR_E_BADARG, "pseudo_nms: null out_count");
    hipStream_t st = semidetr::as_stream(stream);
    if (Q == 0 || C == 0) {
        hipError_t e = hipMemsetAsync(out_count, 0, sizeof(int32_t) * B, st);
        if (e != hipSuccess) return semidetr::fail((int)e, "pseudo_nms memset: %s", hipGetErrorString(e));
        return SEMIDETR_OK;
    }
    SEMIDETR_REQUIRE(max_per_img >= 1 && max_per_img <= kTopCap, SEMIDETR_E_BADARG,
                     "pseudo_nms: max_per_img must be in [1, %d] (got %d)", kTopCap, max_per_img);
    SEMIDETR_REQUIRE(cls_logits && bbox_pred && img_hw && out_dets && out_labels && workspace, SEMIDETR_E_BADARG,
                     "pseudo_nms: null pointer argument");
    SEMIDETR_REQUIRE(iou_thr >= 0.f, SEMIDETR_E_BADARG, "pseudo_nms: iou_thr must be >= 0 (got %g)", (double)iou_thr);
    SEMIDETR_REQUIRE(Q <= 2048, SEMIDETR_E_TOOLARGE, "pseudo_nms: at most 2048 queries per image (got %d)", Q);
    SEMIDETR_REQUIRE((int64_t)Q * C < (int64_t)0xFFFFFFFF, SEMIDETR_E_TOOLARGE, "pseudo_nms: Q * C too large");
    SEMIDETR_REQUIRE(workspace_bytes_ >= workspace_bytes(B, Q, C), SEMIDETR_E_BADARG,
                     "pseudo_nms: workspace too small (%zu < %zu bytes)", workspace_bytes_, workspace_bytes(B, Q, C));
    SEMIDETR_REQUIRE(((uintptr_t)workspace & 15) == 0, SEMIDETR_E_BADARG, "pseudo_nms: workspace must be 16-byte aligned");
    const Workspace ws = carve(workspace, B, Q, C);
    {
        hipError_t e = hipMemsetAsync(ws.maxc, 0, align256(sizeof(float) * (size_t)B) + sizeof(int) * (size_t)B, st);
        if (e != hipSuccess) return semidetr::fail((int)e, "pseudo_nms memset: %s", hipGetErrorString(e));
    }
    hipLaunchKernelGGL(nms_prepare_kernel, dim3((Q + kPrepQueries - 1) / kPrepQueries, B), dim3(256), 0, st, cls_logits, bbox_pred, img_hw, Q, C,
                       score_thr, ws);
    if (int rc = semidetr::launch_status("nms_prepare_kernel")) return rc;
    if (Q <= 256)
        hipLaunchKernelGGL((nms_class_kernel<256, 1>), dim3(C, B), dim3(64), 0, st, cls_logits, Q, C, score_thr, iou_thr, ws);
    else if (Q <= 1024)
        hipLaunchKernelGGL((nms_class_kernel<1024, 4>), dim3(C, B), dim3(256), 0, st, cls_logits, Q, C, score_thr, iou_thr, ws);
    else
        hipLaunchKernelGGL((nms_class_kernel<2048, 4>), dim3(C, B), dim3(256), 0, st, cls_logits, Q, C, score_thr, iou_thr, ws);
    if (int rc = semidetr::launch_status("nms_class_kernel")) return rc;
    hipLaunchKernelGGL(nms_topk_kernel, dim3(B), dim3(kTopThreads), 0, st, cls_logits, Q, C, max_per_img, ws, out_dets,
                       out_labels, out_count);
    return semidetr::launch_status("nms_topk_kernel");
}

extern "C" int semidetr_transform_bboxes_f32(void *stream, const float *boxes, int box_stride,
                                             const int32_t *box_offsets, const int32_t *box_counts,
                                             int num_images, int max_boxes_per_image, const float *matrices,
                                             const float *out_hw, float *out_boxes)
{
    SEMIDETR_REQUIRE(num_images >= 0 && max_boxes_per_image >= 0, SEMIDETR_E_BADARG, "transform_bboxes: negative size");
    if (num_images == 0 || max_boxes_per_image == 0) return SEMIDETR_OK;
    SEMIDETR_REQUIRE(boxes && box_offsets && matrices && out_hw && out_boxes, SEMIDETR_E_BADARG,
                     "transform_bboxes: null pointer argument");
    SEMIDETR_REQUIRE(box_stride >= 4, SEMIDETR_E_BADARG, "transform_bboxes: box_stride must be >= 4 (got %d)", box_stride);
    hipLaunchKernelGGL(transform_bboxes_kernel, dim3((max_boxes_per_image + 255) / 256, num_images), dim3(256), 0,
                       semidetr::as_stream(stream), boxes, box_stride, box_offsets, box_counts, matrices, out_hw,
                       out_boxes);
    return semidetr::launch_status("transform_bboxes_kernel");
}
```

semi-detr_amd/csrc/pseudo_label.hip:

```cpp
#include <hip/hip_runtime.h>

#include "common.h"

namespace {

__device__ __forceinline__ double block_sum(double v, double *red)
{
#pragma unroll
    for (int s = 32; s > 0; s >>= 1) v += __shfl_xor(v, s, 64);
    __syncthreads();
    if ((threadIdx.x & 63) == 0) red[threadIdx.x >> 6] = v;
    __syncthreads();
    return red[0] + red[1] + red[2] + red[3];
}

__global__ __launch_bounds__(256) void pseudo_label_kernel(
    const float *__restrict__ prop, const int64_t *__restrict__ labels, const int32_t *__restrict__ offs,
    const int32_t *__restrict__ counts, float *__restrict__ out_boxes, int64_t *__restrict__ out_labels, float *__restrict__ out_scores,
    int32_t *__restrict__ out_keep, int32_t *__restrict__ out_count, float *__restrict__ out_thr)
{
    __shared__ double red[4];
    __shared__ int wave_cnt[4];
    const int b = blockIdx.x, tid = threadIdx.x;
    const int p0 = offs[b], K = counts ? counts[b] : offs[b + 1] - p0;
    const float *pb = prop + (int64_t)p0 * 5;
    if (K <= 0) {
        if (tid == 0) { out_count[b] = 0; out_thr[b] = __builtin_nanf(""); }
        return;
    }
    double s = 0.0;
    for (int i = tid; i < K; i += 256) s += (double)pb[5 * i + 4];
    const double mean = block_sum(s, red) / K;
    double ss = 0.0;
    for (int i = tid; i < K; i += 256) { const double d = (double)pb[5 * i + 4] - mean; ss += d * d; }
    ss = block_sum(ss, red);
    const float stdv = K > 1 ? (float)sqrt(ss / (K - 1)) : __builtin_nanf("");
    const float thr = __fadd_rn((float)mean, stdv);

    int base = 0;
    for (int i0 = 0; i0 < K; i0 += 256) {
        const int i = i0 + tid;
        bool keep = false;
        float4 box = make_float4(0.f, 0.f, 0.f, 0.f);
        float sc = 0.f;
        if (i < K) {
            box = make_float4(pb[5 * i], pb[5 * i + 1], pb[5 * i + 2], pb[5 * i + 3]);
            sc = pb[5 * i + 4];
            keep = (sc >= thr) && (__fsub_rn(box.z, box.x) > 0.f) && (__fsub_rn(box.w, box.y) > 0.f);
        }
        const unsigned long long mask = __ballot(keep);
        const int lane = tid & 63, wv = tid >> 6;
        const int before = __popcll(mask & ((1ull << lane) - 1ull));
        __syncthreads();
        if (lane == 0) wave_cnt[wv] = __popcll(mask);
        __syncthreads();
        int wbase = 0;
        for (int w = 0; w < wv; ++w) wbase += wave_cnt[w];
        const int total = wave_cnt[0] + wave_cnt[1] + wave_cnt[2] + wave_cnt[3];
        if (keep) {
            const int64_t o = (int64_t)p0 + base + wbase + before;
            out_boxes[4 * o] = box.x; out_boxes[4 * o + 1] = box.y;
            out_boxes[4 * o + 2] = box.z; out_boxes[4 * o + 3] = box.w;
            out_scores[o] = sc;
            if (out_labels) out_labels[o] = labels[p0 + i];
            if (out_keep) out_keep[o] = i;
        }
        base += total;
    }
    if (tid == 0) { out_count[b] = base; out_thr[b] = thr; }
}

}

extern "C" int semidetr_pseudo_label_filter_f32(void *stream, const float *proposals, const int64_t *labels,
                                                const int32_t *prop_offsets, const int32_t *prop_counts,
                                                int num_images, float *out_boxes, int64_t *out_labels, float *out_scores,
                                                int32_t *out_keep_idx, int32_t *out_count, float *out_thr)
{
    SEMIDETR_REQUIRE(num_images >= 0, SEMIDETR_E_BADARG, "pseudo_label: negative num_images");
    if (num_images == 0) return SEMIDETR_OK;
    SEMIDETR_REQUIRE(prop_offsets && out_count && out_thr, SEMIDETR_E_BADARG, "pseudo_label: null pointer argument");
    SEMIDETR_REQUIRE(!out_labels || labels, SEMIDETR_E_BADARG, "pseudo_label: out_labels without labels");
    hipLaunchKernelGGL(pseudo_label_kernel, dim3(num_images), dim3(256), 0, semidetr::as_stream(stream),
                       proposals, labels, prop_offsets, prop_counts, out_boxes, out_labels, out_scores, out_keep_idx,
                       out_count, out_thr);
    return semidetr::launch_status("pseudo_label_kernel");
}
```

semi-detr_amd/matcher.py:

```python
import ctypes

import torch

from . import _lib

_COST_TYPES = {}


def _require_cuda(*tensors):
    for t in tensors:
        if not t.is_cuda:
            raise RuntimeError("semi-detr_amd matcher: tensors must live on the GPU (no CPU fallback)")


class AssignResult:

    def __init__(self, num_gts, gt_inds, max_overlaps, labels=None):
        self.num_gts = num_gts
        self.gt_inds = gt_inds
        self.max_overlaps = max_overlaps
        self.labels = labels
        self._extra_properties = {}

    @property
    def num_preds(self):
        return len(self.gt_inds)

    def __repr__(self):
        return (f"<AssignResult(num_gts={self.num_gts}, gt_inds.shape={tuple(self.gt_inds.shape)}, "
                f"labels.shape={None if self.labels is None else tuple(self.labels.shape)})>")


def _params(cls_weight=0.0, alpha=0.25, gamma=2.0, eps=1e-12, reg_weight=0.0, box_format="xywh",
            iou_weight=0.0, iou_mode="giou", pred_xyxy=False):
    if box_format not in ("xyxy", "xywh"):
        raise AssertionError("box_format must be 'xyxy' or 'xywh'")
    if iou_mode not in ("iou", "giou"):
        raise AssertionError(f"Unsupported mode {iou_mode}")
    return _lib.CostParams(float(cls_weight), float(alpha), float(gamma), float(eps), float(reg_weight),
                           int(box_format == "xywh"), float(iou_weight), int(iou_mode == "giou"),
                           int(bool(pred_xyxy)))


def match_cost_batch(bbox_pred, cls_pred, gt_bboxes, gt_labels, gt_counts, img_wh, params):
    _require_cuda(bbox_pred, cls_pred)
    B, Q, C = cls_pred.shape
    dev = bbox_pred.device
    offs, offs_dev = _lib.offsets(gt_counts, dev)
    total = offs[-1]
    bbox_pred = bbox_pred.detach().to(torch.float32).contiguous()
    cls_pred = cls_pred.detach().to(torch.float32).contiguous()
    gt_bboxes = gt_bboxes.detach().to(device=dev, dtype=torch.float32).reshape(-1, 4).contiguous()
    gt_labels = gt_labels.detach().to(device=dev, dtype=torch.int64).contiguous()
    img_wh = img_wh.to(device=dev, dtype=torch.float32).contiguous()
    cost = torch.empty(Q * total, dtype=torch.float32, device=dev)
    _lib.call("semidetr_match_cost_f32", dev, bbox_pred, cls_pred, gt_bboxes, gt_labels, offs_dev, img_wh, B, Q, C, total,
              ctypes.byref(params), cost)
    return cost, offs_dev, offs


def lsap_batch(cost_flat, offs_dev, offs, Q, gt_labels=None, want_pairs=True, want_assign=True):
    _require_cuda(cost_flat)
    dev = cost_flat.device
    B = len(offs) - 1
    counts = [offs[i + 1] - offs[i] for i in range(B)]
    total, max_gt = offs[-1], max(counts) if counts else 0
    pair_offs = [0]
    for c in counts:
        pair_offs.append(pair_offs[-1] + min(Q, c))
    rows = torch.empty(pair_offs[-1], dtype=torch.int64, device=dev) if want_pairs else None
    cols = torch.empty(pair_offs[-1], dtype=torch.int64, device=dev) if want_pairs else None
    gt_inds = torch.empty((B, Q), dtype=torch.int64, device=dev) if want_assign else None
    labels = torch.empty((B, Q), dtype=torch.int64, device=dev) if want_assign and gt_labels is not None else None
    status = torch.empty(B, dtype=torch.int32, device=dev)
    ws_bytes = _lib.lib().semidetr_lsap_workspace_bytes(B, Q, max_gt)
    ws = torch.empty(ws_bytes, dtype=torch.uint8, device=dev) if ws_bytes else None
    if gt_labels is not None:
        gt_labels = gt_labels.detach().to(device=dev, dtype=torch.int64).contiguous()
    _lib.call("semidetr_lsap_solve", dev, cost_flat, offs_dev, gt_labels, B, Q, total, max_gt, rows, cols, gt_inds, labels,
              status, ws)
    return dict(rows=rows, cols=cols, pair_offsets=pair_offs, gt_inds=gt_inds, labels=labels, status=status)


def raise_on_status(status):
    bad = status.nonzero()
    if bad.numel():
        code = int(status[bad[0, 0]])
        raise ValueError("cost matrix is infeasible" if code == 1 else "matrix contains invalid numeric entries")


def linear_sum_assignment(cost_matrix, maximize=False):
    if maximize:
        raise NotImplementedError("maximize=True is not used on the Semi-DETR path")
    if cost_matrix.dim() != 2:
        raise ValueError("expected a matrix (2-D array), got a %r array" % (tuple(cost_matrix.shape),))
    _require_cuda(cost_matrix)
    Q, G = cost_matrix.shape
    dev = cost_matrix.device
    if Q == 0 or G == 0:
        e = torch.zeros(0, dtype=torch.int64, device=dev)
        return e, e.clone()
    if cost_matrix.dtype != torch.float32:
        raise TypeError("semi-detr_amd linear_sum_assignment takes the fp32 cost matrix the matcher builds")
    flat = cost_matrix.detach().t().contiguous().view(-1)
    offs, offs_dev = _lib.offsets([G], dev)
    res = lsap_batch(flat, offs_dev, offs, Q, want_assign=False)
    raise_on_status(res["status"])
    return res["rows"], res["cols"]


def _dummy_boxes(n, dev):
    b = torch.zeros((n, 4), dtype=torch.float32, device=dev)
    b[:, 2:] = 1.0
    return b


class BBoxL1Cost:

    def __init__(self, weight=1.0, box_format="xyxy"):
        self.weight = weight
        assert box_format in ["xyxy", "xywh"]
        self.box_format = box_format

    def __call__(self, bbox_pred, gt_bboxes):
        Q, G, dev = bbox_pred.size(0), gt_bboxes.size(0), bbox_pred.device
        prm = _params(reg_weight=self.weight, box_format=self.box_format)
        one = torch.ones((1, 2), dtype=torch.float32, device=dev)
        cost, _, _ = match_cost_batch(bbox_pred[None], torch.zeros((1, Q, 1), device=dev), gt_bboxes,
                                      torch.zeros(G, dtype=torch.int64, device=dev), [G], one, prm)
        return cost.view(G, Q).t()


class FocalLossCost:

    def __init__(self, weight=1.0, alpha=0.25, gamma=2, eps=1e-12):
        self.weight, self.alpha, self.gamma, self.eps = weight, alpha, gamma, eps

    def __call__(self, cls_pred, gt_labels):
        Q, G, dev = cls_pred.size(0), gt_labels.size(0), cls_pred.device
        prm = _params(cls_weight=self.weight, alpha=self.alpha, gamma=self.gamma, eps=self.eps)
        one = torch.ones((1, 2), dtype=torch.float32, device=dev)
        cost, _, _ = match_cost_batch(_dummy_boxes(Q, dev)[None], cls_pred[None], _dummy_boxes(G, dev), gt_labels,
                                      [G], one, prm)
        return cost.view(G, Q).t()


class IoUCost:

    def __init__(self, iou_mode="giou", weight=1.0):
        self.weight, self.iou_mode = weight, iou_mode

    def __call__(self, bboxes, gt_bboxes):
        Q, G, dev = bboxes.size(0), gt_bboxes.size(0), bboxes.device
        prm = _params(iou_weight=self.weight, iou_mode=self.iou_mode, pred_xyxy=True)
        one = torch.ones((1, 2), dtype=torch.float32, device=dev)
        cost, _, _ = match_cost_batch(bboxes[None], torch.zeros((1, Q, 1), device=dev), gt_bboxes,
                                      torch.zeros(G, dtype=torch.int64, device=dev), [G], one, prm)
        return cost.view(G, Q).t()


_COST_TYPES.update(BBoxL1Cost=BBoxL1Cost, FocalLossCost=FocalLossCost, IoUCost=IoUCost)


def build_match_cost(cfg):
    if not isinstance(cfg, dict):
        return cfg
    args = dict(cfg)
    typ = args.pop("type")
    if typ not in _COST_TYPES:
        raise KeyError(f"{typ} is not in the match cost registry of semi-detr_amd "
                       f"(supported: {sorted(_COST_TYPES)})")
    return _COST_TYPES[typ](**args)


class HungarianAssigner:

    def __init__(self, cls_cost=dict(type="ClassificationCost", weight=1.0),
                 reg_cost=dict(type="BBoxL1Cost", weight=1.0),
                 iou_cost=dict(type="IoUCost", iou_mode="giou", weight=1.0), debug=False):
        self.cls_cost = build_match_cost(cls_cost)
        self.reg_cost = build_match_cost(reg_cost)
        self.iou_cost = build_match_cost(iou_cost)
        if not isinstance(self.cls_cost, FocalLossCost):
            raise TypeError("semi-detr_amd HungarianAssigner implements the DINO/Semi-DETR configuration "
                            "(FocalLossCost + BBoxL1Cost + IoUCost)")
        self.debug = debug

    def _cost_params(self):
        c, r, i = self.cls_cost, self.reg_cost, self.iou_cost
        return _params(c.weight, c.alpha, c.gamma, c.eps, r.weight, r.box_format, i.weight, i.iou_mode)

    def assign_batch(self, bbox_preds, cls_preds, gt_bboxes_list, gt_labels_list, img_metas, check=True,
                     return_cost=False):
        B, Q = bbox_preds.shape[0], bbox_preds.shape[1]
        dev = bbox_preds.device
        counts = [int(g.size(0)) for g in gt_bboxes_list]
        gt_b = torch.cat([g.reshape(-1, 4) for g in gt_bboxes_list]) if B else bbox_preds.new_zeros((0, 4))
        gt_l = torch.cat([g.reshape(-1).long() for g in gt_labels_list]) if B else bbox_preds.new_zeros(0).long()
        wh = _lib.small_to_device([[m["img_shape"][1], m["img_shape"][0]] for m in img_metas], torch.float32, dev)
        cost, offs_dev, offs = match_cost_batch(bbox_preds, cls_preds, gt_b, gt_l, counts, wh,
                                                self._cost_params())
        res = lsap_batch(cost, offs_dev, offs, Q, gt_labels=gt_l, want_pairs=return_cost)
        if check:
            raise_on_status(res["status"])
        out = []
        for b in range(B):
            gi, lab = res["gt_inds"][b], res["labels"][b]
            if Q == 0:
                gi, lab = gi.new_full((0,), -1), lab.new_full((0,), -1)
            out.append(AssignResult(counts[b], gi, None, labels=lab))
        if return_cost:
            costs = [cost[Q * offs[b]:Q * offs[b + 1]].view(counts[b], Q).t() for b in range(B)]
            return out, costs, res
        return out

    def get_targets_batch(self, bbox_preds, cls_preds, gt_bboxes_list, gt_labels_list, img_metas, num_classes,
                          check=True):
        B, Q = bbox_preds.shape[0], bbox_preds.shape[1]
        dev = bbox_preds.device
        counts = [int(g.size(0)) for g in gt_bboxes_list]
        gt_b = torch.cat([g.reshape(-1, 4) for g in gt_bboxes_list]).to(torch.float32).contiguous()
        gt_l = torch.cat([g.reshape(-1).long() for g in gt_labels_list]).contiguous()
        wh = _lib.small_to_device([[m["img_shape"][1], m["img_shape"][0]] for m in img_metas], torch.float32, dev)
        cost, offs_dev, offs = match_cost_batch(bbox_preds, cls_preds, gt_b, gt_l, counts, wh, self._cost_params())
        res = lsap_batch(cost, offs_dev, offs, Q, gt_labels=gt_l, want_pairs=False)
        labels = torch.empty((B, Q), dtype=torch.int64, device=dev)
        label_weights = torch.empty((B, Q), dtype=torch.float32, device=dev)
        bbox_targets = torch.empty((B, Q, 4), dtype=torch.float32, device=dev)
        bbox_weights = torch.empty((B, Q, 4), dtype=torch.float32, device=dev)
        num_pos = torch.empty(B, dtype=torch.int32, device=dev)
        _lib.call("semidetr_build_targets", dev, res["gt_inds"], gt_b, gt_l, offs_dev, wh, B, Q, int(num_classes), labels,
                  label_weights, bbox_targets, bbox_weights, num_pos)
        if check:
            raise_on_status(res["status"])
        return dict(labels=labels, label_weights=label_weights, bbox_targets=bbox_targets,
                    bbox_weights=bbox_weights, num_pos=num_pos, gt_inds=res["gt_inds"], status=res["status"])

    def assign(self, bbox_pred, cls_pred, gt_bboxes, gt_labels, img_meta, gt_bboxes_ignore=None, eps=1e-7):
        assert gt_bboxes_ignore is None, "Only case when gt_bboxes_ignore is None is supported."
        return self.assign_batch(bbox_pred[None], cls_pred[None], [gt_bboxes], [gt_labels], [img_meta])[0]


class O2MAssignResult:

    def __init__(self, num_gts, gt_inds, max_overlaps, assign_metrics, labels=None):
        self.num_gts = num_gts
        self.gt_inds = gt_inds
        self.max_overlaps = max_overlaps
        self.assign_metrics = assign_metrics
        self.labels = labels
        self._extra_properties = {}

    @property
    def num_preds(self):
        return len(self.gt_inds)

    def __repr__(self):
        return (f"<O2MAssignResult(num_gts={self.num_gts}, gt_inds.shape={tuple(self.gt_inds.shape)}, "
                f"max_overlaps.shape={tuple(self.max_overlaps.shape)})>")


class O2MAssigner:

    def __init__(self, candidate_topk=13, debug=False):
        self.candidate_topk = candidate_topk
        self.debug = debug

    def assign_batch(self, bbox_preds, cls_probs, gt_bboxes_list, gt_labels_list, img_metas, alpha=1, beta=6,
                     candidate_topk=None, dynamic_k=False):
        _require_cuda(bbox_preds, cls_probs)
        B, Q, C = cls_probs.shape
        dev = bbox_preds.device
        k = self.candidate_topk if candidate_topk is None else candidate_topk
        counts = [int(g.size(0)) for g in gt_bboxes_list]
        assert len(counts) == len(gt_labels_list) == len(img_metas) == B
        bp = bbox_preds.detach().to(torch.float32).contiguous()
        cp = cls_probs.detach().to(torch.float32).contiguous()
        gt_b = (torch.cat([g.reshape(-1, 4) for g in gt_bboxes_list]) if B else bp.new_zeros((0, 4)))
        gt_b = gt_b.detach().to(device=dev, dtype=torch.float32).contiguous()
        gt_l = (torch.cat([g.reshape(-1).long() for g in gt_labels_list]) if B else bp.new_zeros(0).long())
        gt_l = gt_l.detach().to(device=dev).contiguous()
        offs, offs_dev = _lib.offsets(counts, dev)
        wh = _lib.small_to_device([[m["img_shape"][1], m["img_shape"][0]] for m in img_metas] or [[1, 1]], torch.float32, dev)
        out = dict(gt_inds=torch.empty((B, Q), dtype=torch.int64, device=dev),
                   labels=torch.empty((B, Q), dtype=torch.int64, device=dev),
                   max_overlaps=torch.empty((B, Q), dtype=torch.float32, device=dev),
                   assign_metrics=torch.empty((B, Q), dtype=torch.float32, device=dev),
                   labels_full=torch.empty((B, Q), dtype=torch.int64, device=dev),
                   bbox_targets=torch.empty((B, Q, 4), dtype=torch.float32, device=dev),
                   norm_metrics=torch.empty((B, Q), dtype=torch.float32, device=dev))
        _lib.call("semidetr_o2m_assign_f32", dev, bp, cp, gt_b, gt_l, offs_dev, wh, B, Q, C, offs[-1],
                  max(counts) if counts else 0, int(k), int(bool(dynamic_k)), float(alpha), float(beta),
                  out["gt_inds"], out["labels"], out["max_overlaps"], out["assign_metrics"], out["labels_full"],
                  out["bbox_targets"], out["norm_metrics"])
        out["num_gts"] = counts
        return out

    def assign(self, bbox_pred, cls_pred, gt_bboxes, gt_labels, img_meta, gt_bboxes_ignore=None, alpha=1, beta=6,
               teacher_assign=False, multiple_pos=False):
        assert gt_bboxes_ignore is None, "Only case when gt_bboxes_ignore is None is supported."
        k = 1 if (teacher_assign and not multiple_pos) else self.candidate_topk
        r = self.assign_batch(bbox_pred[None], cls_pred[None], [gt_bboxes], [gt_labels], [img_meta], alpha, beta, k,
                              dynamic_k=bool(teacher_assign and multiple_pos))
        return O2MAssignResult(r["num_gts"][0], r["gt_inds"][0], r["max_overlaps"][0], r["assign_metrics"][0],
                               labels=r["labels"][0])
```

semi-detr_amd/pseudo_label.py:

```python
import torch

from . import _lib


def filter_pseudo_labels(proposal_box_list, proposal_label_list, return_threshold=False):
    B = len(proposal_box_list)
    if B == 0:
        return ([], [], []) + (([],) if return_threshold else ())
    dev = proposal_box_list[0].device
    if not dev.type == "cuda":
        raise RuntimeError("filter_pseudo_labels: tensors must live on the GPU (no CPU fallback)")
    offs, offs_dev = _lib.offsets([int(p.size(0)) for p in proposal_box_list], dev)
    total = offs[-1]
    prop = torch.cat([p.reshape(-1, 5) for p in proposal_box_list]).to(torch.float32).contiguous()
    lab = torch.cat([l.reshape(-1) for l in proposal_label_list]).to(torch.int64).contiguous()
    out_boxes = torch.empty((total, 4), dtype=torch.float32, device=dev)
    out_labels = torch.empty(total, dtype=torch.int64, device=dev)
    out_scores = torch.empty(total, dtype=torch.float32, device=dev)
    out_keep = torch.empty(total, dtype=torch.int32, device=dev)
    out_count = torch.empty(B, dtype=torch.int32, device=dev)
    out_thr = torch.empty(B, dtype=torch.float32, device=dev)
    _lib.call("semidetr_pseudo_label_filter_f32", dev, prop, lab, offs_dev, None, B, out_boxes, out_labels, out_scores,
              out_keep, out_count, out_thr)
    kept = out_count.tolist()
    det_bboxes = [out_boxes[offs[b]:offs[b] + kept[b]] for b in range(B)]
    det_labels = [out_labels[offs[b]:offs[b] + kept[b]].to(proposal_label_list[b].dtype) for b in range(B)]
    det_scores = [out_scores[offs[b]:offs[b] + kept[b]] for b in range(B)]
    if return_threshold:
        return det_bboxes, det_labels, det_scores, out_thr
    return det_bboxes, det_labels, det_scores


def _img_hw(img_metas, dev):
    return _lib.small_to_device([[float(m["img_shape"][0]), float(m["img_shape"][1])] for m in img_metas], torch.float32, dev)


def _nms_batch(cls_scores, bbox_preds, img_metas, score_thr, iou_threshold, max_per_img):
    if cls_scores.device.type != "cuda":
        raise RuntimeError("get_bboxes_for_pseudo_label: tensors must live on the GPU (no CPU fallback)")
    if cls_scores.dim() != 3 or bbox_preds.shape != cls_scores.shape[:2] + (4,):
        raise ValueError(f"expected cls_scores (B,Q,C) and bbox_preds (B,Q,4), got {tuple(cls_scores.shape)} "
                         f"and {tuple(bbox_preds.shape)}")
    B, Q, C = cls_scores.shape
    assert len(img_metas) == B
    dev = cls_scores.device
    logits = cls_scores.detach().to(torch.float32).contiguous()
    boxes = bbox_preds.detach().to(torch.float32).contiguous()
    hw = _img_hw(img_metas, dev)
    ws = torch.empty(max(int(_lib.lib().semidetr_nms_workspace_bytes(B, Q, C)), 16), dtype=torch.uint8, device=dev)
    dets = torch.empty((B, max_per_img, 5), dtype=torch.float32, device=dev)
    labels = torch.empty((B, max_per_img), dtype=torch.int64, device=dev)
    count = torch.empty(B, dtype=torch.int32, device=dev)
    _lib.call("semidetr_pseudo_nms_f32", dev, logits, boxes, hw, B, Q, C, float(score_thr), float(iou_threshold),
              int(max_per_img), ws, ws.numel(), dets, labels, count)
    return dets, labels, count


def get_bboxes_for_pseudo_label(cls_scores, bbox_preds, img_metas, score_thr=0.01, iou_threshold=0.6,
                                max_per_img=300):
    dets, labels, count = _nms_batch(cls_scores, bbox_preds, img_metas, score_thr, iou_threshold, max_per_img)
    kept = count.tolist()
    return [(dets[b, :kept[b]], labels[b, :kept[b]]) for b in range(len(kept))]


class PendingPseudoLabels:

    def __init__(self, dets, labels, out_boxes, out_labels, out_scores, counts, max_per_img):
        self._t = (dets, labels, out_boxes, out_labels, out_scores)
        self._max = max_per_img
        self._host = torch.empty(tuple(counts.shape), dtype=torch.int32).pin_memory()
        self._host.copy_(counts, non_blocking=True)
        self._event = torch.cuda.Event()
        self._event.record()
        self._lists = None

    def result(self, return_proposals=False):
        if self._lists is None:
            self._event.synchronize()
            both = self._host.tolist()
            dets, labels, ob, ol, os_ = self._t
            m, B = self._max, dets.shape[0]
            self._lists = ([ob[b * m:b * m + both[1][b]] for b in range(B)],
                           [ol[b * m:b * m + both[1][b]] for b in range(B)],
                           [os_[b * m:b * m + both[1][b]] for b in range(B)],
                           [(dets[b, :both[0][b]], labels[b, :both[0][b]]) for b in range(B)])
        return self._lists if return_proposals else self._lists[:3]


def teacher_pseudo_labels(cls_scores, bbox_preds, img_metas, score_thr=0.01, iou_threshold=0.6, max_per_img=300,
                          return_proposals=False, wait=True):
    dets, labels, count = _nms_batch(cls_scores, bbox_preds, img_metas, score_thr, iou_threshold, max_per_img)
    B, dev = dets.shape[0], dets.device
    offs = _lib.small_to_device([b * max_per_img for b in range(B + 1)], torch.int32, dev)
    out_boxes = torch.empty((B * max_per_img, 4), dtype=torch.float32, device=dev)
    out_labels = torch.empty(B * max_per_img, dtype=torch.int64, device=dev)
    out_scores = torch.empty(B * max_per_img, dtype=torch.float32, device=dev)
    out_count = torch.empty(B, dtype=torch.int32, device=dev)
    out_thr = torch.empty(B, dtype=torch.float32, device=dev)
    _lib.call("semidetr_pseudo_label_filter_f32", dev, dets, labels, offs, count, B, out_boxes, out_labels, out_scores,
              None, out_count, out_thr)
    pending = PendingPseudoLabels(dets, labels, out_boxes, out_labels, out_scores, torch.stack([count, out_count]),
                                  max_per_img)
    return pending.result(return_proposals) if wait else pending


def transform_bboxes(bbox, M, out_shape):
    single = isinstance(bbox, torch.Tensor)
    boxes = [bbox] if single else list(bbox)
    mats = [M] if single else list(M)
    shapes = [out_shape] if single else list(out_shape)
    assert len(boxes) == len(mats) == len(shapes)
    B = len(boxes)
    if B == 0:
        return []
    dev = boxes[0].device
    if dev.type != "cuda":
        raise RuntimeError("transform_bboxes: tensors must live on the GPU (no CPU fallback)")
    counts = [int(b.shape[0]) for b in boxes]
    out_list = [b for b in boxes]
    if sum(counts):
        offs, offs_dev = _lib.offsets(counts, dev)
        cat = torch.cat([b[:, :4].to(torch.float32) for b in boxes]).contiguous()
        mt = torch.stack([m.to(device=dev, dtype=torch.float32).reshape(3, 3) for m in mats]).contiguous()
        hw = _lib.small_to_device([[float(s[0]), float(s[1])] for s in shapes], torch.float32, dev)
        out = torch.empty((offs[-1], 4), dtype=torch.float32, device=dev)
        _lib.call("semidetr_transform_bboxes_f32", dev, cat, 4, offs_dev, None, B, max(counts), mt, hw, out)
        out_list = []
        for b in range(B):
            o = out[offs[b]:offs[b + 1]].to(boxes[b].dtype)
            if counts[b] and boxes[b].shape[1] > 4:
                o = torch.cat([o, boxes[b][:, 4:]], dim=1)
            out_list.append(o if counts[b] else boxes[b])
    return out_list[0] if single else out_list
```

Baseline: 455.3.

## Pass per-image metadata as kernel-argument tables to fuse Hungarian and pseudo-label chains

Adds by-value tables (per-image pointers, counts, offsets, image sizes) passed as kernel arguments. A fused Hungarian entry point runs match cost, LSAP and target building in one call, and a native teacher pseudo-label chain and a table-driven box transform are added too. The aim is to remove host-side torch.cat of ground truths, small host-to-device copies of offsets and sizes, and several separate launches from the step. The cost is templated kernels, alignment and dtype checks with fallback paths, and a hard limit of 64 images.

```diff
diff --git a/include/semidetr_hip.h b/include/semidetr_hip.h
--- a/include/semidetr_hip.h
+++ b/include/semidetr_hip.h
@@ -158,6 +158,22 @@
                            int num_problems, int num_query, int64_t num_classes, int64_t *labels,
                            float *label_weights, float *bbox_targets, float *bbox_weights, int32_t *num_pos);
 
+#define SEMIDETR_MATCH_TABLE 64
+typedef struct semidetr_match_table {
+    int num_problems;
+    int32_t count[SEMIDETR_MATCH_TABLE];
+    int32_t offsets[SEMIDETR_MATCH_TABLE + 1];
+    float img_wh[SEMIDETR_MATCH_TABLE][2];
+    const float *boxes[SEMIDETR_MATCH_TABLE];
+    const int64_t *labels[SEMIDETR_MATCH_TABLE];
+} semidetr_match_table;
+int semidetr_hungarian_assign_f32(void *stream, const float *bbox_pred, const float *cls_pred,
+                                  const semidetr_match_table *table , int num_query, int num_classes,
+                                  const semidetr_cost_params *params , float *cost, int64_t *match_row,
+                                  int64_t *match_col, int64_t *assigned_gt_inds, int64_t *assigned_labels, int32_t *status,
+                                  void *workspace, int64_t target_num_classes, int64_t *target_labels, float *label_weights,
+                                  float *bbox_targets, float *bbox_weights, int32_t *num_pos);
+
 #define SEMIDETR_EMA_CHUNK 8192
 int semidetr_ema_multi_f32(void *stream, float *const *teacher_ptrs, const float *const *student_ptrs,
                            const int64_t *numels, const int32_t *block_starts, int num_tensors,
@@ -180,6 +196,27 @@
 int semidetr_transform_bboxes_f32(void *stream, const float *boxes, int box_stride, const int32_t *box_offsets,
                                   const int32_t *box_counts, int num_images, int max_boxes_per_image,
                                   const float *matrices, const float *out_hw, float *out_boxes);
+
+#define SEMIDETR_IMAGE_TABLE 64
+typedef struct semidetr_image_sizes {
+    int num_images;
+    float hw[SEMIDETR_IMAGE_TABLE][2];
+} semidetr_image_sizes;
+typedef struct semidetr_box_table {
+    int num_images;
+    int32_t count[SEMIDETR_IMAGE_TABLE];
+    int32_t box_stride[SEMIDETR_IMAGE_TABLE];
+    int32_t out_offset[SEMIDETR_IMAGE_TABLE];
+    float out_hw[SEMIDETR_IMAGE_TABLE][2];
+    const float *boxes[SEMIDETR_IMAGE_TABLE];
+    const float *matrix[SEMIDETR_IMAGE_TABLE];
+} semidetr_box_table;
+int semidetr_teacher_pseudo_labels_f32(void *stream, const float *cls_logits, const float *bbox_pred,
+                                       const semidetr_image_sizes *img_hw , int num_query, int num_classes,
+                                       float score_thr, float iou_thr, int max_per_img, void *workspace, size_t workspace_bytes,
+                                       float *out_dets, int64_t *out_det_labels, float *out_boxes, int64_t *out_labels,
+                                       float *out_scores, int32_t *counts, float *out_thr);
+int semidetr_transform_bboxes_table_f32(void *stream, const semidetr_box_table *table , float *out_boxes);
 
 int semidetr_o2m_assign_f32(void *stream, const float *bbox_pred, const float *cls_prob, const float *gt_bboxes,
                             const int64_t *gt_labels, const int32_t *gt_offsets, const float *img_wh,
diff --git a/semi-detr_amd/_lib.py b/semi-detr_amd/_lib.py
--- a/semi-detr_amd/_lib.py
+++ b/semi-detr_amd/_lib.py
@@ -36,6 +36,27 @@
                 + _f(c_int, "iou_giou pred_xyxy"))
 
 
+MATCH_TABLE = 64
+
+
+class MatchTable(ctypes.Structure):
+    _fields_ = (_f(c_int, "num_problems") + _f(ctypes.c_int32 * MATCH_TABLE, "count") + _f(ctypes.c_int32 * (MATCH_TABLE + 1), "offsets")
+                + _f(c_float * 2 * MATCH_TABLE, "img_wh") + _f(c_void_p * MATCH_TABLE, "boxes labels"))
+
+
+IMAGE_TABLE = 64
+_IMG_I32 = ctypes.c_int32 * IMAGE_TABLE
+
+
+class ImageSizes(ctypes.Structure):
+    _fields_ = _f(c_int, "num_images") + _f(c_float * 2 * IMAGE_TABLE, "hw")
+
+
+class BoxTable(ctypes.Structure):
+    _fields_ = (_f(c_int, "num_images") + _f(_IMG_I32, "count box_stride out_offset") + _f(c_float * 2 * IMAGE_TABLE, "out_hw")
+                + _f(c_void_p * IMAGE_TABLE, "boxes matrix"))
+
+
 class SetLossSegment(ctypes.Structure):
     _fields_ = (_f(c_int, "kind num_layers num_images num_query num_classes")
                 + _f(c_void_p, "logits") + _f(c_int64 * 3, "logit_stride") + _f(c_void_p, "boxes") + _f(c_int64 * 3, "box_stride")
@@ -127,7 +148,8 @@
                 + _f(RefSegment * REF_MAX_SEGMENTS, "segment"))
 
 
-STRUCTS = {"semidetr_cost_params": CostParams, "semidetr_set_loss_segment": SetLossSegment, "semidetr_dn_layout": DnLayout,
+STRUCTS = {"semidetr_cost_params": CostParams, "semidetr_match_table": MatchTable, "semidetr_image_sizes": ImageSizes,
+           "semidetr_box_table": BoxTable, "semidetr_set_loss_segment": SetLossSegment, "semidetr_dn_layout": DnLayout,
            "semidetr_dn_build": DnBuild, "semidetr_dn_consistency": DnConsistency, "semidetr_consis_layer": ConsisLayer,
            "semidetr_consis_loss": ConsisLoss, "semidetr_self_attn": SelfAttn, "semidetr_self_attn_h16": SelfAttnH16,
            "semidetr_add_norm": AddNorm,
@@ -173,6 +195,8 @@
     "semidetr_lsap_workspace_bytes": (c_int64, [c_int, c_int, c_int]),
     "semidetr_lsap_solve": (c_int, [c_void_p] * 4 + [c_int] * 4 + [c_void_p] * 6),
     "semidetr_build_targets": (c_int, [c_void_p] * 6 + [c_int, c_int, c_int64] + [c_void_p] * 5),
+    "semidetr_hungarian_assign_f32": (c_int, [c_void_p] * 3 + [POINTER(MatchTable), c_int, c_int, POINTER(CostParams)]
+                                      + [c_void_p] * 7 + [c_int64] + [c_void_p] * 5),
     "semidetr_ema_multi_f32": (c_int, [c_void_p] * 5 + [c_int, c_int, c_double]),
     "semidetr_ema_flat_f32": (c_int, [c_void_p, c_void_p, c_void_p, c_int64, c_double]),
     "semidetr_pseudo_label_filter_f32": (c_int, [c_void_p] * 5 + [c_int] + [c_void_p] * 6),
@@ -183,6 +207,9 @@
     "semidetr_tal_loss_workspace_bytes": (c_size_t, []),
     "semidetr_tal_loss_f32": (c_int, [c_void_p] * 4 + [c_int64, c_int, c_float, c_int] + [c_void_p] * 3),
     "semidetr_transform_bboxes_f32": (c_int, [c_void_p, c_void_p, c_int, c_void_p, c_void_p, c_int, c_int] + [c_void_p] * 3),
+    "semidetr_teacher_pseudo_labels_f32": (c_int, [c_void_p] * 3 + [POINTER(ImageSizes), c_int, c_int, c_float, c_float, c_int,
+                                                    c_void_p, c_size_t] + [c_void_p] * 7),
+    "semidetr_transform_bboxes_table_f32": (c_int, [c_void_p, POINTER(BoxTable), c_void_p]),
     "semidetr_gmm_match_costs_f32": (c_int, [c_void_p] * 6 + [c_int] * 4 + [c_void_p] * 2),
     "semidetr_gmm_fit_f64": (c_int, [c_void_p, c_void_p, c_int64, c_void_p, c_int64] + [c_int] * 3 + [c_double, c_double, c_int]
                              + [c_void_p] * 4),
diff --git a/semi-detr_amd/csrc/hungarian_assign.hip b/semi-detr_amd/csrc/hungarian_assign.hip
--- /dev/null
+++ b/semi-detr_amd/csrc/hungarian_assign.hip
@@ -0,0 +1,54 @@
+#include <hip/hip_runtime.h>
+
+#include "common.h"
+#include "match_table.h"
+
+extern "C" int semidetr_hungarian_assign_f32(void *stream, const float *bbox_pred, const float *cls_pred,
+                                             const semidetr_match_table *table, int num_query, int num_classes,
+                                             const semidetr_cost_params *params, float *cost, int64_t *match_row,
+                                             int64_t *match_col, int64_t *assigned_gt_inds, int64_t *assigned_labels,
+                                             int32_t *status, void *workspace, int64_t target_num_classes, int64_t *target_labels,
+                                             float *label_weights, float *bbox_targets, float *bbox_weights, int32_t *num_pos)
+{
+    SEMIDETR_REQUIRE(table && params, SEMIDETR_E_BADARG, "hungarian_assign: null table / params");
+    const int B = table->num_problems;
+    SEMIDETR_REQUIRE(B >= 1 && B <= SEMIDETR_MATCH_TABLE, SEMIDETR_E_BADARG,
+                     "hungarian_assign: %d problems (1 .. %d fit the table)", B, SEMIDETR_MATCH_TABLE);
+    SEMIDETR_REQUIRE(num_query >= 0 && num_classes > 0, SEMIDETR_E_BADARG, "hungarian_assign: bad sizes (Q=%d C=%d)", num_query,
+                     num_classes);
+    int64_t total = 0;
+    int max_gt = 0;
+    for (int b = 0; b < B; ++b) {
+        const int n = table->count[b];
+        SEMIDETR_REQUIRE(n >= 0 && table->offsets[b] == total, SEMIDETR_E_BADARG,
+                         "hungarian_assign: problem %d: count %d, offset %d (expected %lld)", b, n, table->offsets[b],
+                         (long long)total);
+        SEMIDETR_REQUIRE(n == 0 || (table->boxes[b] && table->labels[b]), SEMIDETR_E_BADARG,
+                         "hungarian_assign: problem %d: null boxes / labels", b);
+        SEMIDETR_REQUIRE(((uintptr_t)table->boxes[b] & 15) == 0 && ((uintptr_t)table->labels[b] & 7) == 0, SEMIDETR_E_BADARG,
+                         "hungarian_assign: problem %d: boxes must be 16-byte, labels 8-byte aligned", b);
+        total += n;
+        max_gt = n > max_gt ? n : max_gt;
+        SEMIDETR_REQUIRE((int64_t)num_query * total < INT32_MAX, SEMIDETR_E_TOOLARGE, "hungarian_assign: matrix too large");
+    }
+    SEMIDETR_REQUIRE(table->offsets[B] == total, SEMIDETR_E_BADARG, "hungarian_assign: offsets[%d] = %d, the counts sum to %lld", B,
+                     table->offsets[B], (long long)total);
+    SEMIDETR_REQUIRE(status, SEMIDETR_E_BADARG, "hungarian_assign: null status");
+    const bool has_cost = num_query > 0 && total > 0;
+    SEMIDETR_REQUIRE(!has_cost || (bbox_pred && cls_pred && cost), SEMIDETR_E_BADARG, "hungarian_assign: null pointer argument");
+    SEMIDETR_REQUIRE(((uintptr_t)bbox_pred & 15) == 0, SEMIDETR_E_BADARG, "hungarian_assign: bbox_pred must be 16-byte aligned");
+    if (target_labels)
+        SEMIDETR_REQUIRE(assigned_gt_inds && label_weights && bbox_targets && bbox_weights && num_pos, SEMIDETR_E_BADARG,
+                         "hungarian_assign: targets need assigned_gt_inds and all five target outputs");
+    hipStream_t st = semidetr::as_stream(stream);
+    if (has_cost)
+        if (int rc = semidetr::launch_match_cost_table(st, bbox_pred, cls_pred, *table, num_query, num_classes, *params, cost))
+            return rc;
+    if (int rc = semidetr::launch_lsap_table(st, cost, *table, num_query, max_gt, match_row, match_col, assigned_gt_inds,
+                                             assigned_labels, status, workspace))
+        return rc;
+    if (target_labels)
+        return semidetr::launch_build_targets_table(st, assigned_gt_inds, *table, num_query, target_num_classes, target_labels,
+                                                    label_weights, bbox_targets, bbox_weights, num_pos);
+    return SEMIDETR_OK;
+}
diff --git a/semi-detr_amd/csrc/lsap.hip b/semi-detr_amd/csrc/lsap.hip
--- a/semi-detr_amd/csrc/lsap.hip
+++ b/semi-detr_amd/csrc/lsap.hip
@@ -1,6 +1,7 @@
 #include <hip/hip_runtime.h>
 
 #include "common.h"
+#include "match_table.h"
 
 #pragma clang fp contract(off)
 
@@ -73,16 +74,15 @@
            align16((size_t)nrmax * 4) + align16((size_t)(nrmax + 1) * 4);
 }
 
-template <bool USE_LDS, bool COST_LDS = false>
+template <class GT, bool USE_LDS, bool COST_LDS = false>
 __global__ __launch_bounds__(64) void lsap_kernel(
-    const float *__restrict__ cost, const int32_t *__restrict__ gt_offsets,
-    const int64_t *__restrict__ gt_labels, int Q, int ncmax, int nrmax, int64_t *__restrict__ match_row,
+    const float *__restrict__ cost, const GT gts, int Q, int ncmax, int nrmax, int64_t *__restrict__ match_row,
     int64_t *__restrict__ match_col, int64_t *__restrict__ gt_inds, int64_t *__restrict__ labels,
     int32_t *__restrict__ status, char *__restrict__ ws, size_t ws_stride)
 {
     extern __shared__ double smem_d[];
     const int b = blockIdx.x, lane = threadIdx.x;
-    const int g0 = gt_offsets[b], G = gt_offsets[b + 1] - g0;
+    const int g0 = gts.start(b), G = gts.count(b);
 
     for (int q = lane; q < Q; q += 64) {
         if (gt_inds) gt_inds[(int64_t)b * Q + q] = 0;
@@ -92,7 +92,7 @@
     if (G <= 0 || Q <= 0) return;
 
     int po = 0;
-    for (int bb = lane; bb < b; bb += 64) po += min(Q, gt_offsets[bb + 1] - gt_offsets[bb]);
+    for (int bb = lane; bb < b; bb += 64) po += min(Q, gts.count(bb));
     po = wave_sum_i(po);
 
     const bool tr = G < Q;
@@ -232,7 +232,7 @@
         if (match_row) match_row[po + rank] = q;
         if (match_col) match_col[po + rank] = g;
         if (gt_inds) gt_inds[(int64_t)b * Q + q] = g + 1;
-        if (labels) labels[(int64_t)b * Q + q] = gt_labels[g0 + g];
+        if (labels) labels[(int64_t)b * Q + q] = gts.labels(b)[g];
     }
 }
 
@@ -240,10 +240,9 @@
 constexpr size_t kLdsBig = 150 * 1024;
 
 #pragma clang fp contract(off)
+template <class GT>
 __global__ __launch_bounds__(256) void build_targets_kernel(
-    const int64_t *__restrict__ gt_inds, const float *__restrict__ gt_bboxes, const int64_t *__restrict__ gt_labels,
-    const int32_t *__restrict__ gt_offsets, const float *__restrict__ img_wh, int Q, int64_t num_classes,
-    int64_t *__restrict__ labels, float *__restrict__ label_weights, float *__restrict__ bbox_targets,
+    const int64_t *__restrict__ gt_inds, const GT gts, int Q, int64_t num_classes, int64_t *__restrict__ labels, float *__restrict__ label_weights, float *__restrict__ bbox_targets,
     float *__restrict__ bbox_weights, int32_t *__restrict__ num_pos)
 {
     const int b = blockIdx.y, q = blockIdx.x * 256 + threadIdx.x;
@@ -255,12 +254,12 @@
         float4 t = make_float4(0.f, 0.f, 0.f, 0.f);
         int64_t lab = num_classes;
         if (pos) {
-            const int64_t g = gt_offsets[b] + gi - 1;
-            const float4 bx = *reinterpret_cast<const float4 *>(gt_bboxes + g * 4);
-            const float w = img_wh[2 * b], h = img_wh[2 * b + 1];
+            const int64_t g = gi - 1;
+            const float4 bx = *reinterpret_cast<const float4 *>(gts.boxes(b) + g * 4);
+            const float w = gts.img_w(b), h = gts.img_h(b);
             const float x1 = bx.x / w, y1 = bx.y / h, x2 = bx.z / w, y2 = bx.w / h;
             t = make_float4((x1 + x2) / 2, (y1 + y2) / 2, x2 - x1, y2 - y1);
-            lab = gt_labels[g];
+            lab = gts.labels(b)[g];
         }
         labels[o] = lab;
         label_weights[o] = 1.f;
@@ -270,6 +269,47 @@
     }
     const int n = __popcll(__ballot(pos));
     if ((threadIdx.x & 63) == 0 && n) atomicAdd(&num_pos[b], n);
+}
+
+template <class GT>
+int launch_build_targets(hipStream_t st, const int64_t *assigned_gt_inds, const GT &gts, int num_problems, int num_query,
+                         int64_t num_classes, int64_t *labels, float *label_weights, float *bbox_targets, float *bbox_weights,
+                         int32_t *num_pos)
+{
+    hipError_t e = hipMemsetAsync(num_pos, 0, sizeof(int32_t) * (size_t)num_problems, st);
+    if (e != hipSuccess) return semidetr::fail((int)e, "build_targets memset: %s", hipGetErrorString(e));
+    if (num_query == 0) return SEMIDETR_OK;
+    hipLaunchKernelGGL(build_targets_kernel<GT>, dim3((num_query + 255) / 256, num_problems), dim3(256), 0, st,
+                       assigned_gt_inds, gts, num_query, num_classes, labels, label_weights, bbox_targets, bbox_weights, num_pos);
+    return semidetr::launch_status("build_targets_kernel");
+}
+
+template <class GT>
+int launch_lsap(hipStream_t st, const float *cost, const GT &gts, int num_problems, int num_query, int max_gt,
+                int64_t *match_row, int64_t *match_col, int64_t *assigned_gt_inds, int64_t *assigned_labels, int32_t *status,
+                void *workspace)
+{
+    const int ncmax = num_query > max_gt ? num_query : max_gt;
+    const int nrmax = num_query < max_gt ? num_query : max_gt;
+    const size_t per = lsap_bytes(ncmax > 0 ? ncmax : 1, nrmax > 0 ? nrmax : 1);
+    const size_t cost_bytes = (size_t)max_gt * (size_t)num_query * sizeof(float);
+    if (per <= kLdsLimit && per + cost_bytes <= kLdsBig) {
+        if (int rc = semidetr::allow_big_lds(&lsap_kernel<GT, true, true>, kLdsBig, "lsap")) return rc;
+        hipLaunchKernelGGL((lsap_kernel<GT, true, true>), dim3(num_problems), dim3(64), per + cost_bytes, st, cost, gts,
+                           num_query, ncmax, nrmax, match_row, match_col, assigned_gt_inds,
+                           assigned_labels, status, (char *)nullptr, (size_t)0);
+    } else if (per <= kLdsLimit) {
+        hipLaunchKernelGGL((lsap_kernel<GT, true>), dim3(num_problems), dim3(64), per, st, cost, gts,
+                           num_query, ncmax, nrmax, match_row, match_col, assigned_gt_inds,
+                           assigned_labels, status, (char *)nullptr, (size_t)0);
+    } else {
+        SEMIDETR_REQUIRE(workspace, SEMIDETR_E_BADARG, "lsap: workspace of %lld bytes required",
+                         (long long)(per * (size_t)num_problems));
+        hipLaunchKernelGGL((lsap_kernel<GT, false>), dim3(num_problems), dim3(64), 0, st, cost, gts,
+                           num_query, ncmax, nrmax, match_row, match_col, assigned_gt_inds,
+                           assigned_labels, status, (char *)workspace, per);
+    }
+    return semidetr::launch_status("lsap_kernel");
 }
 
 }
@@ -296,28 +336,9 @@
     SEMIDETR_REQUIRE(gt_offsets && status, SEMIDETR_E_BADARG, "lsap: null gt_offsets/status");
     SEMIDETR_REQUIRE(total_gt == 0 || num_query == 0 || cost, SEMIDETR_E_BADARG, "lsap: null cost");
     SEMIDETR_REQUIRE(!assigned_labels || total_gt == 0 || gt_labels, SEMIDETR_E_BADARG, "lsap: null gt_labels");
-    const int ncmax = num_query > max_gt ? num_query : max_gt;
-    const int nrmax = num_query < max_gt ? num_query : max_gt;
-    const size_t per = lsap_bytes(ncmax > 0 ? ncmax : 1, nrmax > 0 ? nrmax : 1);
-    hipStream_t st = semidetr::as_stream(stream);
-    const size_t cost_bytes = (size_t)max_gt * (size_t)num_query * sizeof(float);
-    if (per <= kLdsLimit && per + cost_bytes <= kLdsBig) {
-        if (int rc = semidetr::allow_big_lds(&lsap_kernel<true, true>, kLdsBig, "lsap")) return rc;
-        hipLaunchKernelGGL((lsap_kernel<true, true>), dim3(num_problems), dim3(64), per + cost_bytes, st, cost, gt_offsets,
-                           gt_labels, num_query, ncmax, nrmax, match_row, match_col, assigned_gt_inds,
-                           assigned_labels, status, (char *)nullptr, (size_t)0);
-    } else if (per <= kLdsLimit) {
-        hipLaunchKernelGGL(lsap_kernel<true>, dim3(num_problems), dim3(64), per, st, cost, gt_offsets,
-                           gt_labels, num_query, ncmax, nrmax, match_row, match_col, assigned_gt_inds,
-                           assigned_labels, status, (char *)nullptr, (size_t)0);
-    } else {
-        SEMIDETR_REQUIRE(workspace, SEMIDETR_E_BADARG, "lsap: workspace of %lld bytes required",
-                         (long long)(per * (size_t)num_problems));
-        hipLaunchKernelGGL(lsap_kernel<false>, dim3(num_problems), dim3(64), 0, st, cost, gt_offsets,
-                           gt_labels, num_query, ncmax, nrmax, match_row, match_col, assigned_gt_inds,
-                           assigned_labels, status, (char *)workspace, per);
-    }
-    return semidetr::launch_status("lsap_kernel");
+    const semidetr::FlatGt gts = {nullptr, gt_labels, gt_offsets, nullptr};
+    return launch_lsap(semidetr::as_stream(stream), cost, gts, num_problems, num_query, max_gt, match_row, match_col,
+                       assigned_gt_inds, assigned_labels, status, workspace);
 }
 
 extern "C" int semidetr_build_targets(void *stream, const int64_t *assigned_gt_inds, const float *gt_bboxes,
@@ -332,12 +353,23 @@
                          bbox_weights && num_pos,
                      SEMIDETR_E_BADARG, "build_targets: null pointer argument");
     SEMIDETR_REQUIRE(num_problems <= 65535, SEMIDETR_E_TOOLARGE, "build_targets: more than 65535 problems");
-    hipStream_t st = semidetr::as_stream(stream);
-    hipError_t e = hipMemsetAsync(num_pos, 0, sizeof(int32_t) * (size_t)num_problems, st);
-    if (e != hipSuccess) return semidetr::fail((int)e, "build_targets memset: %s", hipGetErrorString(e));
-    if (num_query == 0) return SEMIDETR_OK;
-    hipLaunchKernelGGL(build_targets_kernel, dim3((num_query + 255) / 256, num_problems), dim3(256), 0, st,
-                       assigned_gt_inds, gt_bboxes, gt_labels, gt_offsets, img_wh, num_query, num_classes, labels,
-                       label_weights, bbox_targets, bbox_weights, num_pos);
-    return semidetr::launch_status("build_targets_kernel");
-}
+    const semidetr::FlatGt gts = {gt_bboxes, gt_labels, gt_offsets, img_wh};
+    return launch_build_targets(semidetr::as_stream(stream), assigned_gt_inds, gts, num_problems, num_query, num_classes, labels,
+                                label_weights, bbox_targets, bbox_weights, num_pos);
+}
+
+int semidetr::launch_lsap_table(hipStream_t st, const float *cost, const semidetr_match_table &table, int num_query, int max_gt,
+                                int64_t *match_row, int64_t *match_col, int64_t *assigned_gt_inds, int64_t *assigned_labels,
+                                int32_t *status, void *workspace)
+{
+    return launch_lsap(st, cost, semidetr::TableGt{table}, table.num_problems, num_query, max_gt, match_row, match_col,
+                       assigned_gt_inds, assigned_labels, status, workspace);
+}
+
+int semidetr::launch_build_targets_table(hipStream_t st, const int64_t *assigned_gt_inds, const semidetr_match_table &table,
+                                         int num_query, int64_t num_classes, int64_t *labels, float *label_weights,
+                                         float *bbox_targets, float *bbox_weights, int32_t *num_pos)
+{
+    return launch_build_targets(st, assigned_gt_inds, semidetr::TableGt{table}, table.num_problems, num_query, num_classes, labels,
+                                label_weights, bbox_targets, bbox_weights, num_pos);
+}
diff --git a/semi-detr_amd/csrc/match_cost.hip b/semi-detr_amd/csrc/match_cost.hip
--- a/semi-detr_amd/csrc/match_cost.hip
+++ b/semi-detr_amd/csrc/match_cost.hip
@@ -1,6 +1,7 @@
 #include <hip/hip_runtime.h>
 
 #include "common.h"
+#include "match_table.h"
 
 #pragma clang fp contract(off)
 
@@ -11,17 +12,18 @@
     return gamma == 2.0f ? x * x : powf(x, gamma);
 }
 
+template <class GT>
 __global__ __launch_bounds__(256) void match_cost_kernel(
-    const float *__restrict__ bbox_pred, const float *__restrict__ cls_pred,
-    const float *__restrict__ gt_bboxes, const int64_t *__restrict__ gt_labels,
-    const int32_t *__restrict__ gt_offsets, const float *__restrict__ img_wh, int Q, int C,
+    const float *__restrict__ bbox_pred, const float *__restrict__ cls_pred, const GT gts, int Q, int C,
     semidetr_cost_params prm, float *__restrict__ cost)
 {
     const int b = blockIdx.y;
-    const int g0 = gt_offsets[b], G = gt_offsets[b + 1] - g0;
+    const int g0 = gts.start(b), G = gts.count(b);
     const int q = blockIdx.x * 256 + threadIdx.x;
-    if (G <= 0 || q >= Q) return;
-    const float img_w = img_wh[2 * b], img_h = img_wh[2 * b + 1];
+    if (G <= (int)blockIdx.z || q >= Q) return;
+    const float img_w = gts.img_w(b), img_h = gts.img_h(b);
+    const float *__restrict__ gt_bboxes = gts.boxes(b);
+    const int64_t *__restrict__ gt_labels = gts.labels(b);
     const float4 bp = *reinterpret_cast<const float4 *>(bbox_pred + ((int64_t)b * Q + q) * 4);
     float cx = bp.x, cy = bp.y, bw = bp.z, bh = bp.w;
     float nx0 = cx - 0.5f * bw, ny0 = cy - 0.5f * bh, nx1 = cx + 0.5f * bw, ny1 = cy + 0.5f * bh;
@@ -33,9 +35,9 @@
     const float area1 = (x1 - x0) * (y1 - y0);
     const float *cls_row = cls_pred + ((int64_t)b * Q + q) * C;
     float *out = cost + (int64_t)Q * g0 + q;
-    for (int j = 0; j < G; ++j) {
-        const float4 gt = *reinterpret_cast<const float4 *>(gt_bboxes + (int64_t)(g0 + j) * 4);
-        const int label = (int)gt_labels[g0 + j];
+    for (int j = blockIdx.z; j < G; j += gridDim.z) {
+        const float4 gt = *reinterpret_cast<const float4 *>(gt_bboxes + (int64_t)j * 4);
+        const int label = (int)gt_labels[j];
         const float x = (unsigned)label < (unsigned)C ? cls_row[label] : __builtin_nanf("");
         const float p = 1.0f / (1.0f + expf(-x));
         const float neg = -logf(1.0f - p + prm.eps) * (1.0f - prm.alpha) * pow_gamma(p, prm.gamma);
@@ -67,6 +69,12 @@
     }
 }
 
+constexpr int kGtSlices = 16;
+inline dim3 cost_grid(int num_query, int num_problems, int64_t most_gt)
+{
+    return dim3((num_query + 255) / 256, num_problems, (unsigned)(most_gt < kGtSlices ? (most_gt > 0 ? most_gt : 1) : kGtSlices));
+}
+
 }
 
 extern "C" int semidetr_match_cost_f32(void *stream, const float *bbox_pred, const float *cls_pred,
@@ -86,9 +94,21 @@
     SEMIDETR_REQUIRE((int64_t)num_query * total_gt < INT32_MAX, SEMIDETR_E_TOOLARGE, "match_cost: matrix too large");
     SEMIDETR_REQUIRE((((uintptr_t)bbox_pred | (uintptr_t)gt_bboxes) & 15) == 0, SEMIDETR_E_BADARG,
                      "match_cost: bbox_pred / gt_bboxes must be 16-byte aligned");
-    const dim3 grid((num_query + 255) / 256, num_problems);
-    hipLaunchKernelGGL(match_cost_kernel, grid, dim3(256), 0, semidetr::as_stream(stream), bbox_pred,
-                       cls_pred, gt_bboxes, gt_labels, gt_offsets, img_wh, num_query, num_classes, *params,
-                       cost);
+    const dim3 grid = cost_grid(num_query, num_problems, total_gt);
+    const semidetr::FlatGt gts = {gt_bboxes, gt_labels, gt_offsets, img_wh};
+    hipLaunchKernelGGL(match_cost_kernel<semidetr::FlatGt>, grid, dim3(256), 0, semidetr::as_stream(stream), bbox_pred,
+                       cls_pred, gts, num_query, num_classes, *params, cost);
     return semidetr::launch_status("match_cost_kernel");
 }
+
+int semidetr::launch_match_cost_table(hipStream_t st, const float *bbox_pred, const float *cls_pred,
+                                      const semidetr_match_table &table, int num_query, int num_classes,
+                                      const semidetr_cost_params &params, float *cost)
+{
+    int most_gt = 0;
+    for (int b = 0; b < table.num_problems; ++b) most_gt = table.count[b] > most_gt ? table.count[b] : most_gt;
+    const dim3 grid = cost_grid(num_query, table.num_problems, most_gt);
+    hipLaunchKernelGGL(match_cost_kernel<semidetr::TableGt>, grid, dim3(256), 0, st, bbox_pred, cls_pred,
+                       semidetr::TableGt{table}, num_query, num_classes, params, cost);
+    return semidetr::launch_status("match_cost_kernel");
+}
diff --git a/semi-detr_amd/csrc/match_table.h b/semi-detr_amd/csrc/match_table.h
--- /dev/null
+++ b/semi-detr_amd/csrc/match_table.h
@@ -0,0 +1,40 @@
+#pragma once
+#include "common.h"
+
+namespace semidetr {
+
+struct FlatGt {
+    const float *gt_bboxes;
+    const int64_t *gt_labels;
+    const int32_t *gt_offsets;
+    const float *img_wh;
+    __device__ __forceinline__ int start(int b) const { return gt_offsets[b]; }
+    __device__ __forceinline__ int count(int b) const { return gt_offsets[b + 1] - gt_offsets[b]; }
+    __device__ __forceinline__ const float *boxes(int b) const { return gt_bboxes + (int64_t)gt_offsets[b] * 4; }
+    __device__ __forceinline__ const int64_t *labels(int b) const { return gt_labels + gt_offsets[b]; }
+    __device__ __forceinline__ float img_w(int b) const { return img_wh[2 * b]; }
+    __device__ __forceinline__ float img_h(int b) const { return img_wh[2 * b + 1]; }
+};
+
+struct TableGt {
+    semidetr_match_table t;
+    __device__ __forceinline__ int start(int b) const { return t.offsets[b]; }
+    __device__ __forceinline__ int count(int b) const { return t.count[b]; }
+    __device__ __forceinline__ const float *boxes(int b) const { return t.boxes[b]; }
+    __device__ __forceinline__ const int64_t *labels(int b) const { return t.labels[b]; }
+    __device__ __forceinline__ float img_w(int b) const { return t.img_wh[b][0]; }
+    __device__ __forceinline__ float img_h(int b) const { return t.img_wh[b][1]; }
+};
+
+static_assert(sizeof(semidetr_match_table) + 128 <= 4096, "SEMIDETR_MATCH_TABLE: the table does not fit the kernel arguments");
+
+int launch_match_cost_table(hipStream_t st, const float *bbox_pred, const float *cls_pred, const semidetr_match_table &table,
+                            int num_query, int num_classes, const semidetr_cost_params &params, float *cost);
+int launch_lsap_table(hipStream_t st, const float *cost, const semidetr_match_table &table, int num_query, int max_gt,
+                      int64_t *match_row, int64_t *match_col, int64_t *assigned_gt_inds, int64_t *assigned_labels, int32_t *status,
+                      void *workspace);
+int launch_build_targets_table(hipStream_t st, const int64_t *assigned_gt_inds, const semidetr_match_table &table, int num_query,
+                               int64_t num_classes, int64_t *labels, float *label_weights, float *bbox_targets, float *bbox_weights,
+                               int32_t *num_pos);
+
+}
diff --git a/semi-detr_amd/csrc/nms.hip b/semi-detr_amd/csrc/nms.hip
--- a/semi-detr_amd/csrc/nms.hip
+++ b/semi-detr_amd/csrc/nms.hip
@@ -1,6 +1,7 @@
 #include <hip/hip_runtime.h>
 
 #include "common.h"
+#include "pseudo_chain.h"
 
 #pragma clang fp contract(off)
 
@@ -61,14 +62,14 @@
 }
 
 constexpr int kPrepQueries = 16;
+template <class HW>
 __global__ __launch_bounds__(256) void nms_prepare_kernel(const float *__restrict__ logits,
-                                                          const float *__restrict__ bbox_pred,
-                                                          const float *__restrict__ img_hw, int Q, int C,
+                                                          const float *__restrict__ bbox_pred, const HW hw, int Q, int C,
                                                           float score_thr, Workspace ws)
 {
     __shared__ float red[4];
     const int b = blockIdx.y, lane = threadIdx.x & 63, wv = threadIdx.x >> 6;
-    const float img_h = img_hw[2 * b], img_w = img_hw[2 * b + 1];
+    const float img_h = hw.h(b), img_w = hw.w(b);
     float mx = 0.f;
     for (int r = wv; r < kPrepQueries; r += 4) {
         const int q = blockIdx.x * kPrepQueries + r;
@@ -247,19 +248,37 @@
     if (tid == 0) out_count[b] = nout;
 }
 
-__global__ __launch_bounds__(256) void transform_bboxes_kernel(const float *__restrict__ boxes, int box_stride,
-                                                               const int32_t *__restrict__ offs,
-                                                               const int32_t *__restrict__ counts,
-                                                               const float *__restrict__ mats,
-                                                               const float *__restrict__ out_hw,
-                                                               float *__restrict__ out)
+struct BatchBoxes {
+    const float *boxes;
+    int box_stride;
+    const int32_t *offs, *counts;
+    const float *mats, *out_hw;
+    __device__ __forceinline__ int count(int b) const { return counts ? counts[b] : offs[b + 1] - offs[b]; }
+    __device__ __forceinline__ int out_row(int b) const { return offs[b]; }
+    __device__ __forceinline__ const float *box(int b, int i) const { return boxes + (size_t)(offs[b] + i) * box_stride; }
+    __device__ __forceinline__ const float *matrix(int b) const { return mats + 9 * b; }
+    __device__ __forceinline__ float h(int b) const { return out_hw[2 * b]; }
+    __device__ __forceinline__ float w(int b) const { return out_hw[2 * b + 1]; }
+};
+struct TableBoxes {
+    semidetr_box_table t;
+    __device__ __forceinline__ int count(int b) const { return t.count[b]; }
+    __device__ __forceinline__ int out_row(int b) const { return t.out_offset[b]; }
+    __device__ __forceinline__ const float *box(int b, int i) const { return t.boxes[b] + (size_t)i * t.box_stride[b]; }
+    __device__ __forceinline__ const float *matrix(int b) const { return t.matrix[b]; }
+    __device__ __forceinline__ float h(int b) const { return t.out_hw[b][0]; }
+    __device__ __forceinline__ float w(int b) const { return t.out_hw[b][1]; }
+};
+
+template <class SRC>
+__global__ __launch_bounds__(256) void transform_bboxes_kernel(const SRC src, float *__restrict__ out)
 {
     const int b = blockIdx.y;
-    const int p0 = offs[b], K = counts ? counts[b] : offs[b + 1] - p0;
+    const int p0 = src.out_row(b), K = src.count(b);
     const int i = blockIdx.x * 256 + threadIdx.x;
     if (i >= K) return;
-    const float *M = mats + 9 * b;
-    const float *bx = boxes + (size_t)(p0 + i) * box_stride;
+    const float *M = src.matrix(b);
+    const float *bx = src.box(b, i);
     const float px[4] = {bx[0], bx[2], bx[2], bx[0]}, py[4] = {bx[1], bx[1], bx[3], bx[3]};
     float minx = __builtin_huge_valf(), miny = minx, maxx = -minx, maxy = -minx;
 #pragma unroll
@@ -271,7 +290,7 @@
         minx = fminf(minx, u); maxx = fmaxf(maxx, u);
         miny = fminf(miny, v); maxy = fmaxf(maxy, v);
     }
-    const float oh = out_hw[2 * b], ow = out_hw[2 * b + 1];
+    const float oh = src.h(b), ow = src.w(b);
     float *o = out + (size_t)(p0 + i) * 4;
     o[0] = fminf(fmaxf(minx, 0.f), ow);
     o[1] = fminf(fmaxf(miny, 0.f), oh);
@@ -287,17 +306,17 @@
     return workspace_bytes(batch, num_query, num_classes);
 }
 
-extern "C" int semidetr_pseudo_nms_f32(void *stream, const float *cls_logits, const float *bbox_pred,
-                                       const float *img_hw, int batch, int num_query, int num_classes,
-                                       float score_thr, float iou_thr, int max_per_img, void *workspace,
-                                       size_t workspace_bytes_, float *out_dets, int64_t *out_labels,
-                                       int32_t *out_count)
+namespace {
+
+template <class HW>
+int pseudo_nms(hipStream_t st, const float *cls_logits, const float *bbox_pred, const HW &hw, bool have_hw, int batch,
+               int num_query, int num_classes, float score_thr, float iou_thr, int max_per_img, void *workspace,
+               size_t workspace_bytes_, float *out_dets, int64_t *out_labels, int32_t *out_count)
 {
     const int B = batch, Q = num_query, C = num_classes;
     SEMIDETR_REQUIRE(B >= 0 && Q >= 0 && C >= 0, SEMIDETR_E_BADARG, "pseudo_nms: negative size");
     if (B == 0) return SEMIDETR_OK;
     SEMIDETR_REQUIRE(out_count, SEMIDETR_E_BADARG, "pseudo_nms: null out_count");
-    hipStream_t st = semidetr::as_stream(stream);
     if (Q == 0 || C == 0) {
         hipError_t e = hipMemsetAsync(out_count, 0, sizeof(int32_t) * B, st);
         if (e != hipSuccess) return semidetr::fail((int)e, "pseudo_nms memset: %s", hipGetErrorString(e));
@@ -305,7 +324,7 @@
     }
     SEMIDETR_REQUIRE(max_per_img >= 1 && max_per_img <= kTopCap, SEMIDETR_E_BADARG,
                      "pseudo_nms: max_per_img must be in [1, %d] (got %d)", kTopCap, max_per_img);
-    SEMIDETR_REQUIRE(cls_logits && bbox_pred && img_hw && out_dets && out_labels && workspace, SEMIDETR_E_BADARG,
+    SEMIDETR_REQUIRE(cls_logits && bbox_pred && have_hw && out_dets && out_labels && workspace, SEMIDETR_E_BADARG,
                      "pseudo_nms: null pointer argument");
     SEMIDETR_REQUIRE(iou_thr >= 0.f, SEMIDETR_E_BADARG, "pseudo_nms: iou_thr must be >= 0 (got %g)", (double)iou_thr);
     SEMIDETR_REQUIRE(Q <= 2048, SEMIDETR_E_TOOLARGE, "pseudo_nms: at most 2048 queries per image (got %d)", Q);
@@ -318,8 +337,8 @@
         hipError_t e = hipMemsetAsync(ws.maxc, 0, align256(sizeof(float) * (size_t)B) + sizeof(int) * (size_t)B, st);
         if (e != hipSuccess) return semidetr::fail((int)e, "pseudo_nms memset: %s", hipGetErrorString(e));
     }
-    hipLaunchKernelGGL(nms_prepare_kernel, dim3((Q + kPrepQueries - 1) / kPrepQueries, B), dim3(256), 0, st, cls_logits, bbox_pred, img_hw, Q, C,
-                       score_thr, ws);
+    hipLaunchKernelGGL(nms_prepare_kernel<HW>, dim3((Q + kPrepQueries - 1) / kPrepQueries, B), dim3(256), 0, st, cls_logits,
+                       bbox_pred, hw, Q, C, score_thr, ws);
     if (int rc = semidetr::launch_status("nms_prepare_kernel")) return rc;
     if (Q <= 256)
         hipLaunchKernelGGL((nms_class_kernel<256, 1>), dim3(C, B), dim3(64), 0, st, cls_logits, Q, C, score_thr, iou_thr, ws);
@@ -333,6 +352,42 @@
     return semidetr::launch_status("nms_topk_kernel");
 }
 
+}
+
+extern "C" int semidetr_pseudo_nms_f32(void *stream, const float *cls_logits, const float *bbox_pred,
+                                       const float *img_hw, int batch, int num_query, int num_classes,
+                                       float score_thr, float iou_thr, int max_per_img, void *workspace,
+                                       size_t workspace_bytes_, float *out_dets, int64_t *out_labels,
+                                       int32_t *out_count)
+{
+    return pseudo_nms(semidetr::as_stream(stream), cls_logits, bbox_pred, semidetr::DeviceHw{img_hw}, img_hw != nullptr, batch,
+                      num_query, num_classes, score_thr, iou_thr, max_per_img, workspace, workspace_bytes_, out_dets, out_labels,
+                      out_count);
+}
+
+extern "C" int semidetr_teacher_pseudo_labels_f32(void *stream, const float *cls_logits, const float *bbox_pred,
+                                                  const semidetr_image_sizes *img_hw, int num_query, int num_classes,
+                                                  float score_thr, float iou_thr, int max_per_img, void *workspace,
+                                                  size_t workspace_bytes_, float *out_dets, int64_t *out_det_labels,
+                                                  float *out_boxes, int64_t *out_labels, float *out_scores, int32_t *counts,
+                                                  float *out_thr)
+{
+    SEMIDETR_REQUIRE(img_hw, SEMIDETR_E_BADARG, "teacher_pseudo_labels: null img_hw");
+    const int B = img_hw->num_images;
+    SEMIDETR_REQUIRE(B >= 1 && B <= SEMIDETR_IMAGE_TABLE, SEMIDETR_E_BADARG, "teacher_pseudo_labels: %d images (1 .. %d fit the table)",
+                     B, SEMIDETR_IMAGE_TABLE);
+    SEMIDETR_REQUIRE(counts && out_thr && out_boxes && out_labels && out_scores && out_dets && out_det_labels, SEMIDETR_E_BADARG,
+                     "teacher_pseudo_labels: null pointer argument");
+    SEMIDETR_REQUIRE(max_per_img >= 1 && (int64_t)B * max_per_img < INT32_MAX, SEMIDETR_E_BADARG,
+                     "teacher_pseudo_labels: bad max_per_img (%d)", max_per_img);
+    hipStream_t st = semidetr::as_stream(stream);
+    if (int rc = pseudo_nms(st, cls_logits, bbox_pred, semidetr::ValueHw{*img_hw}, true, B, num_query, num_classes, score_thr,
+                            iou_thr, max_per_img, workspace, workspace_bytes_, out_dets, out_det_labels, counts))
+        return rc;
+    return semidetr::launch_pseudo_filter_padded(st, out_dets, out_det_labels, max_per_img, counts, B, out_boxes, out_labels,
+                                                 out_scores, counts + B, out_thr);
+}
+
 extern "C" int semidetr_transform_bboxes_f32(void *stream, const float *boxes, int box_stride,
                                              const int32_t *box_offsets, const int32_t *box_counts,
                                              int num_images, int max_boxes_per_image, const float *matrices,
@@ -343,8 +398,30 @@
     SEMIDETR_REQUIRE(boxes && box_offsets && matrices && out_hw && out_boxes, SEMIDETR_E_BADARG,
                      "transform_bboxes: null pointer argument");
     SEMIDETR_REQUIRE(box_stride >= 4, SEMIDETR_E_BADARG, "transform_bboxes: box_stride must be >= 4 (got %d)", box_stride);
-    hipLaunchKernelGGL(transform_bboxes_kernel, dim3((max_boxes_per_image + 255) / 256, num_images), dim3(256), 0,
-                       semidetr::as_stream(stream), boxes, box_stride, box_offsets, box_counts, matrices, out_hw,
+    hipLaunchKernelGGL(transform_bboxes_kernel<BatchBoxes>, dim3((max_boxes_per_image + 255) / 256, num_images), dim3(256), 0,
+                       semidetr::as_stream(stream), BatchBoxes{boxes, box_stride, box_offsets, box_counts, matrices, out_hw},
                        out_boxes);
     return semidetr::launch_status("transform_bboxes_kernel");
 }
+
+extern "C" int semidetr_transform_bboxes_table_f32(void *stream, const semidetr_box_table *table, float *out_boxes)
+{
+    SEMIDETR_REQUIRE(table, SEMIDETR_E_BADARG, "transform_bboxes_table: null table");
+    const int B = table->num_images;
+    SEMIDETR_REQUIRE(B >= 1 && B <= SEMIDETR_IMAGE_TABLE, SEMIDETR_E_BADARG,
+                     "transform_bboxes_table: %d images (1 .. %d fit the table)", B, SEMIDETR_IMAGE_TABLE);
+    int max_boxes = 0;
+    for (int b = 0; b < B; ++b) {
+        const int n = table->count[b];
+        SEMIDETR_REQUIRE(n >= 0 && table->out_offset[b] >= 0, SEMIDETR_E_BADARG, "transform_bboxes_table: image %d: count %d, row %d",
+                         b, n, table->out_offset[b]);
+        SEMIDETR_REQUIRE(n == 0 || (table->boxes[b] && table->matrix[b] && table->box_stride[b] >= 4), SEMIDETR_E_BADARG,
+                         "transform_bboxes_table: image %d: null boxes / matrix or a row stride below 4", b);
+        max_boxes = n > max_boxes ? n : max_boxes;
+    }
+    if (max_boxes == 0) return SEMIDETR_OK;
+    SEMIDETR_REQUIRE(out_boxes, SEMIDETR_E_BADARG, "transform_bboxes_table: null out_boxes");
+    hipLaunchKernelGGL(transform_bboxes_kernel<TableBoxes>, dim3((max_boxes + 255) / 256, B), dim3(256), 0,
+                       semidetr::as_stream(stream), TableBoxes{*table}, out_boxes);
+    return semidetr::launch_status("transform_bboxes_kernel");
+}
diff --git a/semi-detr_amd/csrc/pseudo_chain.h b/semi-detr_amd/csrc/pseudo_chain.h
--- /dev/null
+++ b/semi-detr_amd/csrc/pseudo_chain.h
@@ -0,0 +1,36 @@
+#pragma once
+#include "common.h"
+
+namespace semidetr {
+
+struct DeviceHw {
+    const float *img_hw;
+    __device__ __forceinline__ float h(int b) const { return img_hw[2 * b]; }
+    __device__ __forceinline__ float w(int b) const { return img_hw[2 * b + 1]; }
+};
+struct ValueHw {
+    semidetr_image_sizes s;
+    __device__ __forceinline__ float h(int b) const { return s.hw[b][0]; }
+    __device__ __forceinline__ float w(int b) const { return s.hw[b][1]; }
+};
+
+struct DeviceRows {
+    const int32_t *offs, *counts;
+    __device__ __forceinline__ int start(int b) const { return offs[b]; }
+    __device__ __forceinline__ int count(int b) const { return counts ? counts[b] : offs[b + 1] - offs[b]; }
+};
+struct PaddedRows {
+    int stride;
+    const int32_t *counts;
+    __device__ __forceinline__ int start(int b) const { return b * stride; }
+    __device__ __forceinline__ int count(int b) const { return counts[b]; }
+};
+
+static_assert(sizeof(semidetr_box_table) + 64 <= 4096 && sizeof(semidetr_image_sizes) + 128 <= 4096,
+              "SEMIDETR_IMAGE_TABLE: the tables do not fit the kernel arguments");
+
+int launch_pseudo_filter_padded(hipStream_t st, const float *proposals, const int64_t *labels, int stride, const int32_t *counts,
+                                int num_images, float *out_boxes, int64_t *out_labels, float *out_scores, int32_t *out_count,
+                                float *out_thr);
+
+}
diff --git a/semi-detr_amd/csrc/pseudo_label.hip b/semi-detr_amd/csrc/pseudo_label.hip
--- a/semi-detr_amd/csrc/pseudo_label.hip
+++ b/semi-detr_amd/csrc/pseudo_label.hip
@@ -1,6 +1,7 @@
 #include <hip/hip_runtime.h>
 
 #include "common.h"
+#include "pseudo_chain.h"
 
 namespace {
 
@@ -14,15 +15,15 @@
     return red[0] + red[1] + red[2] + red[3];
 }
 
+template <class ROWS>
 __global__ __launch_bounds__(256) void pseudo_label_kernel(
-    const float *__restrict__ prop, const int64_t *__restrict__ labels, const int32_t *__restrict__ offs,
-    const int32_t *__restrict__ counts, float *__restrict__ out_boxes, int64_t *__restrict__ out_labels, float *__restrict__ out_scores,
+    const float *__restrict__ prop, const int64_t *__restrict__ labels, const ROWS rows, float *__restrict__ out_boxes, int64_t *__restrict__ out_labels, float *__restrict__ out_scores,
     int32_t *__restrict__ out_keep, int32_t *__restrict__ out_count, float *__restrict__ out_thr)
 {
     __shared__ double red[4];
     __shared__ int wave_cnt[4];
     const int b = blockIdx.x, tid = threadIdx.x;
-    const int p0 = offs[b], K = counts ? counts[b] : offs[b + 1] - p0;
+    const int p0 = rows.start(b), K = rows.count(b);
     const float *pb = prop + (int64_t)p0 * 5;
     if (K <= 0) {
         if (tid == 0) { out_count[b] = 0; out_thr[b] = __builtin_nanf(""); }
@@ -81,8 +82,18 @@
     if (num_images == 0) return SEMIDETR_OK;
     SEMIDETR_REQUIRE(prop_offsets && out_count && out_thr, SEMIDETR_E_BADARG, "pseudo_label: null pointer argument");
     SEMIDETR_REQUIRE(!out_labels || labels, SEMIDETR_E_BADARG, "pseudo_label: out_labels without labels");
-    hipLaunchKernelGGL(pseudo_label_kernel, dim3(num_images), dim3(256), 0, semidetr::as_stream(stream),
-                       proposals, labels, prop_offsets, prop_counts, out_boxes, out_labels, out_scores, out_keep_idx,
-                       out_count, out_thr);
+    hipLaunchKernelGGL(pseudo_label_kernel<semidetr::DeviceRows>, dim3(num_images), dim3(256), 0, semidetr::as_stream(stream),
+                       proposals, labels, semidetr::DeviceRows{prop_offsets, prop_counts}, out_boxes, out_labels, out_scores,
+                       out_keep_idx, out_count, out_thr);
     return semidetr::launch_status("pseudo_label_kernel");
 }
+
+int semidetr::launch_pseudo_filter_padded(hipStream_t st, const float *proposals, const int64_t *labels, int stride,
+                                          const int32_t *counts, int num_images, float *out_boxes, int64_t *out_labels,
+                                          float *out_scores, int32_t *out_count, float *out_thr)
+{
+    hipLaunchKernelGGL(pseudo_label_kernel<semidetr::PaddedRows>, dim3(num_images), dim3(256), 0, st, proposals, labels,
+                       semidetr::PaddedRows{stride, counts}, out_boxes, out_labels, out_scores, (int32_t *)nullptr, out_count,
+                       out_thr);
+    return semidetr::launch_status("pseudo_label_kernel");
+}
diff --git a/semi-detr_amd/matcher.py b/semi-detr_amd/matcher.py
--- a/semi-detr_amd/matcher.py
+++ b/semi-detr_amd/matcher.py
@@ -82,6 +82,74 @@
     return dict(rows=rows, cols=cols, pair_offsets=pair_offs, gt_inds=gt_inds, labels=labels, status=status)
 
 
+NATIVE_CHAIN = True
+
+
+def pack_match_table(box_ptrs, label_ptrs, counts, img_wh):
+    B = len(counts)
+    if not 1 <= B <= _lib.MATCH_TABLE or not len(box_ptrs) == len(label_ptrs) == len(img_wh) == B:
+        raise ValueError(f"pack_match_table: {B} problems (1 .. {_lib.MATCH_TABLE} fit the table, one entry of each list per problem)")
+    offs = [0]
+    for c in counts:
+        offs.append(offs[-1] + c)
+    t = _lib.MatchTable()
+    t.num_problems = B
+    t.count[:B] = counts
+    t.offsets[:B + 1] = offs
+    t.boxes[:B] = box_ptrs
+    t.labels[:B] = label_ptrs
+    for b, (w, h) in enumerate(img_wh):
+        t.img_wh[b][0], t.img_wh[b][1] = w, h
+    return t, offs
+
+
+def _table_inputs_ok(gt_bboxes_list, gt_labels_list, dev):
+    B = len(gt_bboxes_list)
+    if not NATIVE_CHAIN or not 1 <= B <= _lib.MATCH_TABLE or len(gt_labels_list) != B:
+        return False
+    for g, l in zip(gt_bboxes_list, gt_labels_list):
+        if (g.dtype != torch.float32 or l.dtype != torch.int64 or g.device != dev or l.device != dev or g.dim() != 2
+                or g.size(1) != 4 or l.dim() != 1 or l.size(0) != g.size(0) or not g.is_contiguous() or not l.is_contiguous()
+                or g.data_ptr() % 16 or l.data_ptr() % 8):
+            return False
+    return True
+
+
+def hungarian_assign_batch(bbox_pred, cls_pred, gt_bboxes_list, gt_labels_list, img_metas, params, want_pairs=False,
+                           num_classes=None):
+    _require_cuda(bbox_pred, cls_pred)
+    B, Q, C = cls_pred.shape
+    dev = bbox_pred.device
+    bbox_pred = bbox_pred.detach().to(torch.float32).contiguous()
+    cls_pred = cls_pred.detach().to(torch.float32).contiguous()
+    counts = [g.size(0) for g in gt_bboxes_list]
+    table, offs = pack_match_table([g.data_ptr() for g in gt_bboxes_list], [l.data_ptr() for l in gt_labels_list], counts,
+                                   [(m["img_shape"][1], m["img_shape"][0]) for m in img_metas])
+    total, max_gt = offs[-1], max(counts)
+    pair_offs = [0]
+    for c in counts:
+        pair_offs.append(pair_offs[-1] + min(Q, c))
+    cost = torch.empty(Q * total, dtype=torch.float32, device=dev)
+    rows = torch.empty(pair_offs[-1], dtype=torch.int64, device=dev) if want_pairs else None
+    cols = torch.empty(pair_offs[-1], dtype=torch.int64, device=dev) if want_pairs else None
+    gt_inds = torch.empty((B, Q), dtype=torch.int64, device=dev)
+    labels = torch.empty((B, Q), dtype=torch.int64, device=dev)
+    status = torch.empty(B, dtype=torch.int32, device=dev)
+    ws_bytes = _lib.lib().semidetr_lsap_workspace_bytes(B, Q, max_gt)
+    ws = torch.empty(ws_bytes, dtype=torch.uint8, device=dev) if ws_bytes else None
+    tg = None
+    if num_classes is not None:
+        tg = dict(labels=torch.empty((B, Q), dtype=torch.int64, device=dev),
+                  label_weights=torch.empty((B, Q), dtype=torch.float32, device=dev),
+                  bbox_targets=torch.empty((B, Q, 4), dtype=torch.float32, device=dev),
+                  bbox_weights=torch.empty((B, Q, 4), dtype=torch.float32, device=dev),
+                  num_pos=torch.empty(B, dtype=torch.int32, device=dev))
+    _lib.call("semidetr_hungarian_assign_f32", dev, bbox_pred, cls_pred, ctypes.byref(table), Q, C, ctypes.byref(params), cost,
+              rows, cols, gt_inds, labels, status, ws, int(num_classes or 0), *(tg.values() if tg else (None,) * 5))
+    res = dict(rows=rows, cols=cols, pair_offsets=pair_offs, gt_inds=gt_inds, labels=labels, status=status)
+    return cost, offs, res, tg
+
+
 def raise_on_status(status):
     bad = status.nonzero()
     if bad.numel():
@@ -195,12 +263,16 @@
         B, Q = bbox_preds.shape[0], bbox_preds.shape[1]
         dev = bbox_preds.device
         counts = [int(g.size(0)) for g in gt_bboxes_list]
-        gt_b = torch.cat([g.reshape(-1, 4) for g in gt_bboxes_list]) if B else bbox_preds.new_zeros((0, 4))
-        gt_l = torch.cat([g.reshape(-1).long() for g in gt_labels_list]) if B else bbox_preds.new_zeros(0).long()
-        wh = _lib.small_to_device([[m["img_shape"][1], m["img_shape"][0]] for m in img_metas], torch.float32, dev)
-        cost, offs_dev, offs = match_cost_batch(bbox_preds, cls_preds, gt_b, gt_l, counts, wh,
-                                                self._cost_params())
-        res = lsap_batch(cost, offs_dev, offs, Q, gt_labels=gt_l, want_pairs=return_cost)
+        if len(img_metas) == B and _table_inputs_ok(gt_bboxes_list, gt_labels_list, dev):
+            cost, offs, res, _ = hungarian_assign_batch(bbox_preds, cls_preds, gt_bboxes_list, gt_labels_list, img_metas,
+                                                        self._cost_params(), want_pairs=return_cost)
+        else:
+            gt_b = torch.cat([g.reshape(-1, 4) for g in gt_bboxes_list]) if B else bbox_preds.new_zeros((0, 4))
+            gt_l = torch.cat([g.reshape(-1).long() for g in gt_labels_list]) if B else bbox_preds.new_zeros(0).long()
+            wh = _lib.small_to_device([[m["img_shape"][1], m["img_shape"][0]] for m in img_metas], torch.float32, dev)
+            cost, offs_dev, offs = match_cost_batch(bbox_preds, cls_preds, gt_b, gt_l, counts, wh,
+                                                    self._cost_params())
+            res = lsap_batch(cost, offs_dev, offs, Q, gt_labels=gt_l, want_pairs=return_cost)
         if check:
             raise_on_status(res["status"])
         out = []
@@ -218,6 +290,12 @@
                           check=True):
         B, Q = bbox_preds.shape[0], bbox_preds.shape[1]
         dev = bbox_preds.device
+        if len(img_metas) == B and _table_inputs_ok(gt_bboxes_list, gt_labels_list, dev):
+            _, _, res, tg = hungarian_assign_batch(bbox_preds, cls_preds, gt_bboxes_list, gt_labels_list, img_metas,
+                                                   self._cost_params(), num_classes=int(num_classes))
+            if check:
+                raise_on_status(res["status"])
+            return dict(tg, gt_inds=res["gt_inds"], status=res["status"])
         counts = [int(g.size(0)) for g in gt_bboxes_list]
         gt_b = torch.cat([g.reshape(-1, 4) for g in gt_bboxes_list]).to(torch.float32).contiguous()
         gt_l = torch.cat([g.reshape(-1).long() for g in gt_labels_list]).contiguous()
diff --git a/semi-detr_amd/pseudo_label.py b/semi-detr_amd/pseudo_label.py
--- a/semi-detr_amd/pseudo_label.py
+++ b/semi-detr_amd/pseudo_label.py
@@ -1,6 +1,10 @@
+import ctypes
+
 import torch
 
 from . import _lib
+
+NATIVE_CHAIN = True
 
 
 def filter_pseudo_labels(proposal_box_list, proposal_label_list, return_threshold=False):
@@ -87,8 +91,40 @@
         return self._lists if return_proposals else self._lists[:3]
 
 
+def _teacher_chain(cls_scores, bbox_preds, img_metas, score_thr, iou_threshold, max_per_img):
+    if cls_scores.device.type != "cuda":
+        raise RuntimeError("get_bboxes_for_pseudo_label: tensors must live on the GPU (no CPU fallback)")
+    if bbox_preds.shape != cls_scores.shape[:2] + (4,):
+        raise ValueError(f"expected cls_scores (B,Q,C) and bbox_preds (B,Q,4), got {tuple(cls_scores.shape)} "
+                         f"and {tuple(bbox_preds.shape)}")
+    B, Q, C = cls_scores.shape
+    assert len(img_metas) == B
+    dev = cls_scores.device
+    logits = cls_scores.detach().to(torch.float32).contiguous()
+    boxes = bbox_preds.detach().to(torch.float32).contiguous()
+    hw = _lib.ImageSizes()
+    hw.num_images = B
+    for b, m in enumerate(img_metas):
+        hw.hw[b][0], hw.hw[b][1] = float(m["img_shape"][0]), float(m["img_shape"][1])
+    ws = torch.empty(max(int(_lib.lib().semidetr_nms_workspace_bytes(B, Q, C)), 16), dtype=torch.uint8, device=dev)
+    dets = torch.empty((B, max_per_img, 5), dtype=torch.float32, device=dev)
+    labels = torch.empty((B, max_per_img), dtype=torch.int64, device=dev)
+    out_boxes = torch.empty((B * max_per_img, 4), dtype=torch.float32, device=dev)
+    out_labels = torch.empty(B * max_per_img, dtype=torch.int64, device=dev)
+    out_scores = torch.empty(B * max_per_img, dtype=torch.float32, device=dev)
+    counts = torch.empty((2, B), dtype=torch.int32, device=dev)
+    out_thr = torch.empty(B, dtype=torch.float32, device=dev)
+    _lib.call("semidetr_teacher_pseudo_labels_f32", dev, logits, boxes, ctypes.byref(hw), Q, C, float(score_thr),
+              float(iou_threshold), int(max_per_img), ws, ws.numel(), dets, labels, out_boxes, out_labels, out_scores, counts,
+              out_thr)
+    return PendingPseudoLabels(dets, labels, out_boxes, out_labels, out_scores, counts, max_per_img)
+
+
 def teacher_pseudo_labels(cls_scores, bbox_preds, img_metas, score_thr=0.01, iou_threshold=0.6, max_per_img=300,
                           return_proposals=False, wait=True):
+    if NATIVE_CHAIN and cls_scores.dim() == 3 and 1 <= cls_scores.shape[0] <= _lib.IMAGE_TABLE:
+        pending = _teacher_chain(cls_scores, bbox_preds, img_metas, score_thr, iou_threshold, max_per_img)
+        return pending.result(return_proposals) if wait else pending
     dets, labels, count = _nms_batch(cls_scores, bbox_preds, img_metas, score_thr, iou_threshold, max_per_img)
     B, dev = dets.shape[0], dets.device
     offs = _lib.small_to_device([b * max_per_img for b in range(B + 1)], torch.int32, dev)
@@ -102,6 +138,44 @@
     pending = PendingPseudoLabels(dets, labels, out_boxes, out_labels, out_scores, torch.stack([count, out_count]),
                                   max_per_img)
     return pending.result(return_proposals) if wait else pending
+
+
+def _box_table_ok(boxes, mats, dev):
+    if not NATIVE_CHAIN or not 1 <= len(boxes) <= _lib.IMAGE_TABLE:
+        return False
+    for b, m in zip(boxes, mats):
+        if (b.dtype != torch.float32 or b.device != dev or b.dim() != 2 or b.shape[1] < 4 or b.stride(1) != 1
+                or (b.shape[0] > 1 and b.stride(0) < 4) or b.data_ptr() % 4):
+            return False
+        if (not isinstance(m, torch.Tensor) or m.dtype != torch.float32 or m.device != dev or m.numel() != 9
+                or not m.is_contiguous()):
+            return False
+    return True
+
+
+def _transform_table(boxes, mats, shapes, counts, dev):
+    B = len(boxes)
+    t = _lib.BoxTable()
+    t.num_images = B
+    offs = [0]
+    for c in counts:
+        offs.append(offs[-1] + c)
+    t.count[:B] = counts
+    t.out_offset[:B] = offs[:B]
+    t.box_stride[:B] = [max(int(b.stride(0)), 4) for b in boxes]
+    t.boxes[:B] = [b.data_ptr() for b in boxes]
+    t.matrix[:B] = [m.data_ptr() for m in mats]
+    for b, s in enumerate(shapes):
+        t.out_hw[b][0], t.out_hw[b][1] = float(s[0]), float(s[1])
+    out = torch.empty((offs[-1], 4), dtype=torch.float32, device=dev)
+    _lib.call("semidetr_transform_bboxes_table_f32", dev, ctypes.byref(t), out)
+    out_list = []
+    for b in range(B):
+        o = out[offs[b]:offs[b + 1]]
+        if counts[b] and boxes[b].shape[1] > 4:
+            o = torch.cat([o, boxes[b][:, 4:]], dim=1)
+        out_list.append(o if counts[b] else boxes[b])
+    return out_list
 
 
 def transform_bboxes(bbox, M, out_shape):
@@ -118,7 +192,9 @@
         raise RuntimeError("transform_bboxes: tensors must live on the GPU (no CPU fallback)")
     counts = [int(b.shape[0]) for b in boxes]
     out_list = [b for b in boxes]
-    if sum(counts):
+    if sum(counts) and _box_table_ok(boxes, mats, dev):
+        out_list = _transform_table(boxes, mats, shapes, counts, dev)
+    elif sum(counts):
         offs, offs_dev = _lib.offsets(counts, dev)
         cat = torch.cat([b[:, :4].to(torch.float32) for b in boxes]).contiguous()
         mt = torch.stack([m.to(device=dev, dtype=torch.float32).reshape(3, 3) for m in mats]).contiguous()
```

Result: faster. 460.1, median of 6 (+1.1%).
